# DoHoonKim8/halo2-lasso

Hardware: AMD Instinct MI355X
Metric: lasso_prove_time_ms (lower is better)
Workload: dtype u256 (BN254 Fr/Fq, 8x u32 Montgomery); 1 GPU; 2^24 AND Lasso lookup (32-bit operands, 4 chunks of 8+8 bits); lookups_per_proof=16777216, pcs=multilinear KZG (BN254), proof_bytes=64256, parallelism=1 GPU

## Files before the change

### bindings/rust/src/sys.rs

```rust
#![allow(non_camel_case_types, dead_code)]
use halo2_curves::bn256::{Fr, G1Affine, G2Affine};
use std::os::raw::{c_char, c_int, c_void};

pub type lh_status = c_int;
pub const LH_OK: lh_status = 0;
pub const LH_ERR_INVALID_SUMCHECK: lh_status = -1;
pub const LH_ERR_INVALID_PCS_PARAM: lh_status = -2;
pub const LH_ERR_INVALID_PCS_OPEN: lh_status = -3;
pub const LH_ERR_INVALID_SNARK: lh_status = -4;
pub const LH_ERR_SERIALIZATION: lh_status = -5;
pub const LH_ERR_TRANSCRIPT: lh_status = -6;
pub const LH_ERR_DEVICE: lh_status = -7;
pub const LH_ERR_ARG: lh_status = -8;

pub const LH_SC_MAX_TERMS: usize = 48;
pub const LH_SC_MAX_FACTORS: usize = 4;
pub const LH_SC_EVALUATIONS: c_int = 0;
pub const LH_SC_COEFFICIENTS: c_int = 1;
pub const LH_LASSO_MAX_CHUNKS: usize = 8;
pub const LH_LASSO_MAX_MEMORIES: usize = 16;
pub const LH_LASSO_MAX_TERMS: usize = 16;
pub const LH_RCCL_UNIQUE_ID_BYTES: usize = 128;

#[repr(C)] pub struct lh_ctx { _p: [u8; 0] }
// ... 71 lines not shown
    pub g_num_factors: [u8; LH_LASSO_MAX_TERMS],
    pub g_factor: [[u8; LH_SC_MAX_FACTORS]; LH_LASSO_MAX_TERMS],
}

#[repr(C)]
pub struct lh_comm {
    pub rank: c_int,
    pub size: c_int,
    pub user: *mut c_void,
    pub all_gather: Option<unsafe extern "C" fn(*mut c_void, *const c_void, *mut c_void, usize) -> c_int>,
    pub all_gather_device: Option<unsafe extern "C" fn(*mut c_void, *const c_void, *mut c_void, usize, *mut c_void) -> c_int>,
}

#[repr(C)]
pub struct lh_hp_lookup { pub inputs: *const lh_expr, pub tables: *const lh_expr, pub width: usize }
#[repr(C)] #[derive(Clone, Copy)]
pub struct lh_hp_lasso_lookup {
    pub table: lh_lasso_table,
    pub output_poly: usize,
    pub chunk_polys: [usize; LH_LASSO_MAX_CHUNKS],
}
#[repr(C)]
pub struct lh_hp_param {
    pub num_vars: usize,
    pub num_instance_polys: usize,
    pub num_instances: *const usize,
    pub num_preprocess_polys: usize,
    pub d_preprocess_polys: *const *const c_void,
    pub num_witness_polys: usize,
    pub num_challenges: usize,
    pub num_lookups: usize,
    pub lookups: *const lh_hp_lookup,
    pub num_permutation_polys: usize,
    pub permutation_poly_index: *const usize,
    pub d_permutation_polys: *const *const c_void,
    pub num_permutation_z_polys: usize,
    pub expression: lh_expr,
    pub num_lasso_lookups: usize,
    pub lasso_lookups: *const lh_hp_lasso_lookup,
}
#[repr(C)]
pub struct lh_hp_vparam {
    pub num_vars: usize,
    pub num_instance_polys: usize,
    pub num_instances: *const usize,
    pub num_witness_polys: usize,
    pub num_challenges: usize,
    pub num_lookups: usize,
    pub num_permutation_z_polys: usize,
    pub expression: lh_expr,
    pub num_preprocess_polys: usize,
    pub preprocess_comms: *const G1Affine,
    pub num_permutation_polys: usize,
    pub permutation_comms: *const G1Affine,
    pub num_lasso_lookups: usize,
    pub lasso_lookups: *const lh_hp_lasso_lookup,
}
#[repr(C)]
pub struct lh_hp_circuit {
    pub user: *mut c_void,
    pub synthesize: Option<unsafe extern "C" fn(*mut c_void, usize, *const Fr, usize, *mut *const c_void, usize) -> c_int>,
}

#[repr(C)]
#[derive(Clone, Copy, Debug, Default)]
pub struct lh_lasso_route {
    pub open_small_depth: u32,
    pub open_small_passes: u32,
    pub eq_factored_rounds: u32,
    pub standard_rounds: u32,
    pub rw_leaf_rounds: u32,
    pub resident_tails: u32,
    pub resident_rounds: u32,
    pub packed_ts_pairs: u32,
    pub derived_commitments: u32,
    pub sorted_dim_reuse: u32,
    pub sharded_rounds: u32,
    pub shard_exchanges: u32,
    pub window_table_jobs: u32,
    pub open_precommit: u32,
    pub resident_layers: u32,
    pub pp_folds: u32,
    pub msm_half_batches: u32,
    pub reserved: [u32; 7],
}

extern "C" {
    pub fn lh_last_error() -> *const c_char;
    pub fn lh_version() -> *const c_char;
    pub fn lh_ctx_create(device_id: c_int, out: *mut *mut lh_ctx) -> lh_status;
    pub fn lh_ctx_destroy(ctx: *mut lh_ctx);
    pub fn lh_ctx_sync(ctx: *mut lh_ctx) -> lh_status;
    pub fn lh_ctx_stream(ctx: *mut lh_ctx) -> *mut c_void;
    pub fn lh_alloc(ctx: *mut lh_ctx, bytes: usize, d_out: *mut *mut c_void) -> lh_status;
    pub fn lh_free(ctx: *mut lh_ctx, d_ptr: *mut c_void) -> lh_status;
    pub fn lh_upload(ctx: *mut lh_ctx, d_dst: *mut c_void, src: *const c_void, bytes: usize) -> lh_status;
    pub fn lh_download(ctx: *mut lh_ctx, dst: *mut c_void, d_src: *const c_void, bytes: usize) -> lh_status;
    pub fn lh_fr_from_u64(ctx: *mut lh_ctx, d_in: *const u64, n: usize, d_out: *mut Fr) -> lh_status;
    pub fn lh_fr_from_u32(ctx: *mut lh_ctx, d_in: *const u32, n: usize, d_out: *mut Fr) -> lh_status;
    pub fn lh_fr_batch_invert(ctx: *mut lh_ctx, d_in: *const Fr, n: usize, d_out: *mut Fr) -> lh_status;
    pub fn lh_fix_var(ctx: *mut lh_ctx, d_in: *const Fr, n_in: usize, x: *const Fr, d_out: *mut Fr) -> lh_status;
    pub fn lh_eq_xy(ctx: *mut lh_ctx, y: *const Fr, num_vars: usize, d_out: *mut Fr) -> lh_status;
    pub fn lh_evaluate(ctx: *mut lh_ctx, d_polys: *const *const Fr, num_polys: usize, num_vars: usize,
                       point: *const Fr, out_evals: *mut Fr) -> lh_status;
    pub fn lh_lincomb(ctx: *mut lh_ctx, d_polys: *const *const Fr, w: *const Fr, num_polys: usize, n: usize,
                      d_out: *mut Fr) -> lh_status;
    pub fn lh_sumcheck_prove(ctx: *mut lh_ctx, prover_kind: c_int, num_vars: usize, expr: *const lh_sop,
                             d_polys: *const *const Fr, num_polys: usize, ys: *const Fr, num_ys: usize,
                             sum: *const Fr, t: *mut lh_transcript, out_challenges: *mut Fr, out_evals: *mut Fr) -> lh_status;
    pub fn lh_sumcheck_prove_expr(ctx: *mut lh_ctx, num_vars: usize, expr: *const lh_expr, d_polys: *const *const Fr,
                                  num_polys: usize, challenges: *const Fr, num_challenges: usize, ys: *const Fr,
                                  num_ys: usize, sum: *const Fr, t: *mut lh_transcript, out_challenges: *mut Fr,
                                  out_evals: *mut Fr) -> lh_status;
    pub fn lh_sumcheck_verify(prover_kind: c_int, num_vars: usize, degree: usize, sum: *const Fr,
                              t: *mut lh_transcript, out_eval: *mut Fr, out_x: *mut Fr) -> lh_status;
    pub fn lh_gkr_fractional_prove(ctx: *mut lh_ctx, num_batching: usize, num_vars: usize,
                                   claimed_p_0s: *const *const Fr, claimed_q_0s: *const *const Fr,
                                   d_ps: *const *const Fr, d_qs: *const *const Fr, t: *mut lh_transcript,
                                   out_p_xs: *mut Fr, out_q_xs: *mut Fr, out_x: *mut Fr) -> lh_status;
    pub fn lh_msm(ctx: *mut lh_ctx, d_scalars: *const Fr, d_bases: *const G1Affine, n: usize, out: *mut G1Affine) -> lh_status;
    pub fn lh_msm_u32(ctx: *mut lh_ctx, d_scalars: *const u32, d_bases: *const G1Affine, n: usize, out: *mut G1Affine) -> lh_status;
    pub fn lh_srs_upload(ctx: *mut lh_ctx, eqs_flat: *const G1Affine, num_vars: usize, out: *mut *mut lh_srs) -> lh_status;
    pub fn lh_srs_num_vars(srs: *const lh_srs) -> usize;
    pub fn lh_srs_free(ctx: *mut lh_ctx, srs: *mut lh_srs);
    pub fn lh_mkzg_batch_commit(ctx: *mut lh_ctx, srs: *const lh_srs, d_polys: *const *const Fr, num_polys: usize,
                                num_vars: usize, out_comms: *mut G1Affine) -> lh_status;
    pub fn lh_mkzg_open(ctx: *mut lh_ctx, srs: *const lh_srs, d_poly: *const Fr, num_vars: usize, point: *const Fr,
                        t: *mut lh_transcript, out_eval: *mut Fr) -> lh_status;
    pub fn lh_mkzg_batch_open(ctx: *mut lh_ctx, srs: *const lh_srs, num_vars: usize, d_polys: *const *const Fr,
                              num_polys: usize, points: *const Fr, num_points: usize, evals: *const lh_evaluation,
                              num_evals: usize, t: *mut lh_transcript) -> lh_status;
    pub fn lh_mkzg_vp_new(g1: *const G1Affine, g2: *const G2Affine, ss: *const G2Affine, num_vars: usize,
                          out: *mut *mut lh_mkzg_vp) -> lh_status;
    pub fn lh_mkzg_vp_free(vp: *mut lh_mkzg_vp);
    pub fn lh_mkzg_verify(vp: *const lh_mkzg_vp, comm: *const G1Affine, point: *const Fr, num_vars: usize,
                          eval: *const Fr, t: *mut lh_transcript) -> lh_status;
    pub fn lh_mkzg_batch_verify(vp: *const lh_mkzg_vp, num_vars: usize, comms: *const G1Affine, num_comms: usize,
                                points: *const Fr, num_points: usize, evals: *const lh_evaluation, num_evals: usize,
                                t: *mut lh_transcript) -> lh_status;
    pub fn lh_lasso_prove(ctx: *mut lh_ctx, srs: *const lh_srs, table: *const lh_lasso_table, num_vars: usize,
                          d_dims: *const *const u32, t: *mut lh_transcript) -> lh_status;
    pub fn lh_lasso_verify(vp: *const lh_mkzg_vp, table: *const lh_lasso_table, num_vars: usize,
                           t: *mut lh_transcript) -> lh_status;
    pub fn lh_ctx_set_comm(ctx: *mut lh_ctx, comm: *const lh_comm, shard_bit: usize) -> lh_status;
    pub fn lh_rccl_unique_id(out: *mut u8) -> lh_status;
    pub fn lh_ctx_set_comm_rccl(ctx: *mut lh_ctx, rank: c_int, size: c_int, unique_id: *const u8, shard_bit: usize) -> lh_status;
    pub fn lh_ctx_set_comm_loopback(ctx: *mut lh_ctx, rank: c_int, size: c_int, shard_bit: usize) -> lh_status;
    pub fn lh_ctx_comm_stats(ctx: *mut lh_ctx, out: *mut u64) -> lh_status;
    pub fn lh_ctx_comm_phase_stats(ctx: *mut lh_ctx, out: *mut u64, reset: c_int) -> lh_status;
    pub fn lh_ctx_memory_stats(ctx: *mut lh_ctx, out: *mut u64) -> lh_status;
    pub fn lh_ctx_host_cpus(ctx: *mut lh_ctx, bus_id: *mut c_char, bus_id_cap: usize, cpulist: *mut c_char, cpulist_cap: usize) -> lh_status;
    pub fn lh_shard_extract(ctx: *mut lh_ctx, d_global: *const c_void, n_local: usize, shard_bit: usize, rho: usize,
                            rank: usize, elem_bytes: usize, d_local: *mut c_void) -> lh_status;
    pub fn lh_ctx_set_option(ctx: *mut lh_ctx, name: *const c_char, value: i64) -> lh_status;
    pub fn lh_ctx_get_option(ctx: *mut lh_ctx, name: *const c_char, out: *mut i64) -> lh_status;
    pub fn lh_lasso_last_route(ctx: *mut lh_ctx, out: *mut lh_lasso_route) -> lh_status;
    pub fn lh_lasso_prove_sharded(ctx: *mut lh_ctx, srs: *const lh_srs, table: *const lh_lasso_table, num_vars: usize,
                                  d_dims_local: *const *const u32, t: *mut lh_transcript) -> lh_status;
    pub fn lh_hyperplonk_prove(ctx: *mut lh_ctx, srs: *const lh_srs, pp: *const lh_hp_param,
                               instances: *const *const Fr, d_witness_polys: *const *const Fr,
                               t: *mut lh_transcript) -> lh_status;
    pub fn lh_hyperplonk_prove_sharded(ctx: *mut lh_ctx, srs: *const lh_srs, pp: *const lh_hp_param,
                                       instances: *const *const Fr, d_witness_polys_local: *const *const Fr,
                                       t: *mut lh_transcript) -> lh_status;
    pub fn lh_hyperplonk_prove_phases(ctx: *mut lh_ctx, srs: *const lh_srs, pp: *const lh_hp_param, num_phases: usize,
                                      num_witness_polys: *const usize, num_challenges: *const usize,
                                      instances: *const *const Fr, circuit: *const lh_hp_circuit,
// ... 135 lines not shown
```

### halo2-lasso_amd/__init__.py

```python
import ctypes as C

from . import _ffi
from ._ffi import (lh_fr, lh_g1, lh_sop, lh_evaluation, lh_lasso_table, lh_transcript,
                   LH_SC_EVALUATIONS, LH_SC_COEFFICIENTS)

R_MOD = 0x30644E72E131A029B85045B68181585D2833E84879B9709143E1F593F0000001
Q_MOD = 0x30644E72E131A029B85045B68181585D97816A916871CA8D3C208C16D87CFD47
_MONT = 1 << 256
_MONT_INV_R = pow(_MONT, -1, R_MOD)
_MONT_INV_Q = pow(_MONT, -1, Q_MOD)

SUBTABLE_IDENTITY, SUBTABLE_AND, SUBTABLE_XOR = 0, 1, 2


class Error(Exception):
    code = None


class InvalidSumcheck(Error):
    code = _ffi.LH_ERR_INVALID_SUMCHECK


class InvalidPcsParam(Error):
    code = _ffi.LH_ERR_INVALID_PCS_PARAM
# ... 335 lines not shown
    return _fr_list(out, len(polys))


EvaluationsProver = LH_SC_EVALUATIONS
CoefficientsProver = LH_SC_COEFFICIENTS


class SumOfProducts:

    def __init__(self, terms, global_eq=-1):
        self.terms, self.global_eq = [(c % R_MOD, list(f)) for c, f in terms], global_eq

    def to_c(self):
        s = lh_sop()
        s.num_terms, s.global_eq = len(self.terms), self.global_eq
        for m, (coeff, facs) in enumerate(self.terms):
            C.memmove(C.byref(s.coeff[m]), fr_to_bytes(coeff), 32)
            s.num_factors[m] = len(facs)
            for k, f in enumerate(facs):
                s.factor[m][k] = f
        return s


class ClassicSumCheck:
    @staticmethod
    def prove(ctx, prover, num_vars, expression, polys, ys, sum_, transcript):
        if len(expression.terms) > _ffi.LH_SC_MAX_TERMS:
            raise ArgumentError("too many terms")
        ys_flat = [v for y in ys for v in y]
        ch = (lh_fr * max(num_vars, 1))()
        ev = (lh_fr * max(len(polys), 1))()
        sop = expression.to_c()
        _check(ctx.lib.lh_sumcheck_prove(ctx.h, prover, num_vars, C.byref(sop), _ptr_array(polys), len(polys),
                                         _fr_array(ys_flat), len(ys), _fr_array([sum_]), transcript.p, ch, ev))
        return _fr_list(ch, num_vars), _fr_list(ev, len(polys))


def sum_check_prove_expression(ctx, num_vars, expression, polys, challenges, ys, sum_, transcript):
    ce, keep = expression.to_c()
    ys_flat = [v for y in ys for v in y]
    ch = (lh_fr * max(num_vars, 1))()
    ev = (lh_fr * max(len(polys), 1))()
    _check(ctx.lib.lh_sumcheck_prove_expr(ctx.h, num_vars, C.byref(ce), _ptr_array(polys), len(polys),
                                          _fr_array(challenges), len(challenges), _fr_array(ys_flat), len(ys),
                                          _fr_array([sum_]), transcript.p, ch, ev))
    return _fr_list(ch, num_vars), _fr_list(ev, len(polys))


def prove_fractional_sum_check(ctx, claimed_p_0s, claimed_q_0s, ps, qs, transcript):
    B = len(ps)
    if not (B == len(qs) == len(claimed_p_0s) == len(claimed_q_0s)):
        raise ArgumentError("length mismatch")
    num_vars = ps[0].num_vars if B else 0
    for p in list(ps) + list(qs):
        if p.num_vars != num_vars:
            raise ArgumentError("num_vars mismatch")

    def opt(claims):
        keep = [_fr_array([c]) if c is not None else None for c in claims]
        arr = (C.POINTER(lh_fr) * max(B, 1))()
        for i, k in enumerate(keep):
            arr[i] = C.cast(k, C.POINTER(lh_fr)) if k is not None else None
        return arr, keep

    cp, keep_p = opt(claimed_p_0s)
    cq, keep_q = opt(claimed_q_0s)
    p_xs, q_xs, x = (lh_fr * max(B, 1))(), (lh_fr * max(B, 1))(), (lh_fr * max(num_vars, 1))()
    _check(ctx.lib.lh_gkr_fractional_prove(ctx.h, B, num_vars, cp, cq, _ptr_array(ps), _ptr_array(qs),
                                           transcript.p, p_xs, q_xs, x))
    return _fr_list(p_xs, B), _fr_list(q_xs, B), _fr_list(x, num_vars)


def prove_grand_product(ctx, leaves, transcript):
    B = len(leaves)
    nv = (C.c_size_t * max(B, 1))(*[p.num_vars for p in leaves])
    total = sum(p.num_vars for p in leaves)
    roots, claims, points = (lh_fr * max(B, 1))(), (lh_fr * max(B, 1))(), (lh_fr * max(total, 1))()
    _check(ctx.lib.lh_grand_product_prove(ctx.h, B, _ptr_array(leaves), nv, transcript.p, roots, claims, points))
    pts, flat, off = [], _fr_list(points, total), 0
    for p in leaves:
        pts.append(flat[off:off + p.num_vars])
        off += p.num_vars
    return _fr_list(roots, B), list(zip(_fr_list(claims, B), pts))


def variable_base_msm(ctx, scalars, bases, n=None):
    n = len(scalars) if n is None else n
    out = lh_g1()
    _check(ctx.lib.lh_msm(ctx.h, scalars.ptr, bases.ptr, n, C.byref(out)))
    return g1_from_bytes(bytes(out))


def variable_base_msm_u32(ctx, scalars, bases, n):
    out = lh_g1()
    _check(ctx.lib.lh_msm_u32(ctx.h, scalars.ptr, bases.ptr, n, C.byref(out)))
    return g1_from_bytes(bytes(out))


class Evaluation:

    def __init__(self, poly, point, value):
        self.poly, self.point, self.value = poly, point, value % R_MOD


class MultilinearKzgParams:
    def __init__(self, ctx, handle, borrowed=False):
        self.ctx, self.h, self.borrowed = ctx, handle, borrowed

    def view(self, ctx):
        return MultilinearKzgParams(ctx, self.h, borrowed=True)

    @property
    def num_vars(self):
        return self.ctx.lib.lh_srs_num_vars(self.h)

    def eqs_bytes(self):
        total = (2 << self.num_vars) - 1
        out = C.create_string_buffer(64 * total)
        _check(self.ctx.lib.lh_srs_download(self.ctx.h, self.h, out))
        return out.raw

    def eqs(self):
        n = self.num_vars
        total = (2 << n) - 1
        out = C.create_string_buffer(64 * total)
        _check(self.ctx.lib.lh_srs_download(self.ctx.h, self.h, out))
        pts = [g1_from_bytes(out.raw[64 * i:64 * i + 64]) for i in range(total)]
        return [pts[(1 << k) - 1:(2 << k) - 1] for k in range(n + 1)]

    def free(self):
        if self.h and self.ctx.h and not self.borrowed:
            self.ctx.lib.lh_srs_free(self.ctx.h, self.h)
        self.h = None

    def __del__(self):
        try:
            self.free()
        except Exception:
            pass


class MultilinearKzg:

    @staticmethod
    def setup(ctx, ss):
        h = C.c_void_p()
        _check(ctx.lib.lh_mkzg_setup(ctx.h, _fr_array(ss), len(ss), C.byref(h)))
        return MultilinearKzgParams(ctx, h)

    @staticmethod
    def upload(ctx, eqs_levels):
        flat = b"".join(g1_to_bytes(p) for lvl in eqs_levels for p in lvl)
        return MultilinearKzg.upload_bytes(ctx, flat, len(eqs_levels) - 1)

    @staticmethod
    def upload_bytes(ctx, eqs_flat, num_vars):
        if len(eqs_flat) != 64 * ((2 << num_vars) - 1):
            raise ArgumentError("flat SRS has the wrong length")
        h = C.c_void_p()
        _check(ctx.lib.lh_srs_upload(ctx.h, eqs_flat, num_vars, C.byref(h)))
        return MultilinearKzgParams(ctx, h)

    @staticmethod
    def commit(pp, poly):
        out = lh_g1()
        _check(pp.ctx.lib.lh_mkzg_commit(pp.ctx.h, pp.h, poly.ptr, poly.num_vars, C.byref(out)))
# ... 859 lines not shown
                return _ffi.LH_ERR_ARG
            C.memmove(recv, out, len(out))
            return 0
        except Exception:
            return _ffi.LH_ERR_DEVICE
    comm = _ffi.lh_comm()
    comm.rank, comm.size, comm.user = rank, size, None
    comm.all_gather = _ffi._AG_CB(cb)
    ctx._comm_keepalive = (comm, cb)
    _check(ctx.lib.lh_ctx_set_comm(ctx.h, C.byref(comm), shard_bit))


def rccl_unique_id():
    buf = C.create_string_buffer(_ffi.LH_RCCL_UNIQUE_ID_BYTES)
    _check(_ffi.load().lh_rccl_unique_id(buf))
    return buf.raw


def attach_comm_rccl(ctx, rank, size, unique_id, shard_bit):
    if len(unique_id) != _ffi.LH_RCCL_UNIQUE_ID_BYTES:
        raise ArgumentError("unique id must be %d bytes" % _ffi.LH_RCCL_UNIQUE_ID_BYTES)
    _check(ctx.lib.lh_ctx_set_comm_rccl(ctx.h, rank, size, unique_id, shard_bit))


def comm_stats(ctx):
    out = (C.c_uint64 * 2)()
    _check(ctx.lib.lh_ctx_comm_stats(ctx.h, out))
    return {"device": int(out[0]), "host": int(out[1])}


def comm_phase_stats(ctx, reset=False):
    out = (C.c_uint64 * 16)()
    _check(ctx.lib.lh_ctx_comm_phase_stats(ctx.h, out, 1 if reset else 0))
    names = ["witness", "commit", "surge", "leaves", "gkr", "evals", "open", "outside"]
    return {nm: {"collectives": int(out[2 * i]), "bytes": int(out[2 * i + 1])} for i, nm in enumerate(names) if out[2 * i]}


def memory_stats(ctx):
    out = (C.c_uint64 * 4)()
    _check(ctx.lib.lh_ctx_memory_stats(ctx.h, out))
    return {"arena_high_water_bytes": int(out[0]), "arena_reserved_bytes": int(out[1]), "device_free_bytes": int(out[2]),
            "device_total_bytes": int(out[3])}


def attach_comm_loopback(ctx, rank, size, shard_bit):
    _check(ctx.lib.lh_ctx_set_comm_loopback(ctx.h, rank, size, shard_bit))


def detach_comm(ctx):
    _check(ctx.lib.lh_ctx_set_comm(ctx.h, None, 0))
    ctx._comm_keepalive = None


def shard_of(column, rank, size, shard_bit):
    rho = size.bit_length() - 1
    n = len(column)
    return column.reshape(n >> (shard_bit + rho), size, 1 << shard_bit)[:, rank, :].reshape(-1).copy()


def shard_poly(poly, rank, size, shard_bit):
    rho = size.bit_length() - 1
    n_local = (1 << poly.num_vars) >> rho
    out = poly.ctx.alloc(32 * n_local)
    _check(poly.ctx.lib.lh_shard_extract(poly.ctx.h, poly.ptr, n_local, shard_bit, rho, rank, 32, out.ptr))
    return MultilinearPolynomial(poly.ctx, out, poly.num_vars - rho)


def lasso_prove_sharded(pp, table, num_vars, dims_local, transcript):
    if len(dims_local) != table.c:
        raise ArgumentError("expected %d dim columns" % table.c)
    t = table.to_c()
    _check(pp.ctx.lib.lh_lasso_prove_sharded(pp.ctx.h, pp.h, C.byref(t), num_vars, _ptr_array(dims_local), transcript.p))


def lasso_last_timing(ctx):
    out = (C.c_double * _ffi.LH_LASSO_NUM_PHASES)()
    _check(ctx.lib.lh_lasso_last_timing(ctx.h, out))
    names = ["witness", "commit", "surge", "leaves", "gkr", "evals", "open_n", "open_l", "total"]
    return dict(zip(names, list(out)))


ROUTE_FIELDS = ["open_small_depth", "open_small_passes", "eq_factored_rounds", "standard_rounds", "rw_leaf_rounds",
                "resident_tails", "resident_rounds", "packed_ts_pairs", "derived_commitments", "sorted_dim_reuse",
                "sharded_rounds", "shard_exchanges", "window_table_jobs", "open_precommit", "resident_layers", "pp_folds", "msm_half_batches"]


def lasso_last_route(ctx):
    out = (C.c_uint32 * 24)()
    _check(ctx.lib.lh_lasso_last_route(ctx.h, out))
    return dict(zip(ROUTE_FIELDS, [int(v) for v in out]))


def set_option(ctx, name, value):
    _check(ctx.lib.lh_ctx_set_option(ctx.h, name.encode(), int(value)))


def get_option(ctx, name):
    out = C.c_int64(0)
    _check(ctx.lib.lh_ctx_get_option(ctx.h, name.encode(), C.byref(out)))
    return int(out.value)


def profile_enable(ctx, on=True):
    _check(ctx.lib.lh_profile_enable(ctx.h, int(on)))


def profile_read(ctx):
    n = C.c_size_t()
    _check(ctx.lib.lh_profile_read(ctx.h, None, 0, C.byref(n)))
    arr = (_ffi.lh_prof_rec * max(n.value, 1))()
    _check(ctx.lib.lh_profile_read(ctx.h, arr, n.value, C.byref(n)))
    return [dict(name=r.name.decode(), ms=r.ms, bytes=r.bytes, muls=r.muls, items=r.items) for r in arr[:n.value]]


from . import expression
```

### halo2-lasso_amd/_ffi.py

```python
import ctypes as C
import os

_HERE = os.path.dirname(os.path.abspath(__file__))
LIB_PATH = os.path.join(_HERE, "liblasso_hip.so")

LH_OK = 0
LH_ERR_INVALID_SUMCHECK, LH_ERR_INVALID_PCS_PARAM, LH_ERR_INVALID_PCS_OPEN = -1, -2, -3
LH_ERR_INVALID_SNARK, LH_ERR_SERIALIZATION, LH_ERR_TRANSCRIPT, LH_ERR_DEVICE, LH_ERR_ARG = -4, -5, -6, -7, -8
LH_SC_EVALUATIONS, LH_SC_COEFFICIENTS = 0, 1
LH_SC_MAX_TERMS, LH_SC_MAX_FACTORS = 48, 4
LH_LASSO_MAX_CHUNKS, LH_LASSO_MAX_MEMORIES, LH_LASSO_MAX_TERMS = 8, 16, 16
LH_LASSO_NUM_PHASES = 9


class lh_fr(C.Structure):
    _fields_ = [("l", C.c_uint64 * 4)]


class lh_g1(C.Structure):
    _fields_ = [("x", C.c_uint64 * 4), ("y", C.c_uint64 * 4)]


class lh_sop(C.Structure):
    _fields_ = [("num_terms", C.c_uint32), ("global_eq", C.c_int32),
# ... 62 lines not shown
class lh_evaluation(C.Structure):
    _fields_ = [("poly", C.c_uint32), ("point", C.c_uint32), ("value", lh_fr)]


_AG_CB = C.CFUNCTYPE(C.c_int, C.c_void_p, C.c_void_p, C.c_void_p, C.c_size_t)
_AGD_CB = C.CFUNCTYPE(C.c_int, C.c_void_p, C.c_void_p, C.c_void_p, C.c_size_t, C.c_void_p)
LH_RCCL_UNIQUE_ID_BYTES = 128


class lh_comm(C.Structure):
    _fields_ = [("rank", C.c_int), ("size", C.c_int), ("user", C.c_void_p), ("all_gather", _AG_CB),
                ("all_gather_device", _AGD_CB)]


class lh_prof_rec(C.Structure):
    _fields_ = [("name", C.c_char * 40), ("ms", C.c_double), ("bytes", C.c_double), ("muls", C.c_double),
                ("items", C.c_double)]


_FE_CB = C.CFUNCTYPE(C.c_int, C.c_void_p, C.POINTER(lh_fr))
_G1_CB = C.CFUNCTYPE(C.c_int, C.c_void_p, C.POINTER(lh_g1))


class lh_transcript(C.Structure):
    _fields_ = [("user", C.c_void_p),
                ("write_field_element", _FE_CB), ("common_field_element", _FE_CB),
                ("squeeze_challenge", _FE_CB),
                ("write_commitment", _G1_CB), ("common_commitment", _G1_CB),
                ("read_field_element", _FE_CB), ("read_commitment", _G1_CB)]


_HASH_W_CB = C.CFUNCTYPE(C.c_int, C.c_void_p, C.POINTER(C.c_uint8))


class lh_hash_transcript(C.Structure):
    _fields_ = [("user", C.c_void_p), ("write_hash", _HASH_W_CB), ("read_hash", _HASH_W_CB)]


class lh_g2(C.Structure):
    _fields_ = [("x_c0", C.c_uint64 * 4), ("x_c1", C.c_uint64 * 4), ("y_c0", C.c_uint64 * 4), ("y_c1", C.c_uint64 * 4)]


_P = C.c_void_p
_SZ = C.c_size_t
SIGNATURES = {
    "lh_last_error": (C.c_char_p, []),
    "lh_version": (C.c_char_p, []),
    "lh_ctx_create": (C.c_int, [C.c_int, C.POINTER(_P)]),
    "lh_ctx_destroy": (None, [_P]),
    "lh_ctx_sync": (C.c_int, [_P]),
    "lh_ctx_stream": (_P, [_P]),
    "lh_alloc": (C.c_int, [_P, _SZ, C.POINTER(_P)]),
    "lh_free": (C.c_int, [_P, _P]),
    "lh_upload": (C.c_int, [_P, _P, _P, _SZ]),
    "lh_download": (C.c_int, [_P, _P, _P, _SZ]),
    "lh_keccak_transcript_new": (C.c_int, [C.POINTER(C.POINTER(lh_transcript))]),
    "lh_keccak_transcript_free": (None, [C.POINTER(lh_transcript)]),
    "lh_keccak_transcript_proof": (C.c_int, [C.POINTER(lh_transcript), C.POINTER(C.POINTER(C.c_uint8)),
                                             C.POINTER(_SZ)]),
    "lh_fr_from_u64": (C.c_int, [_P, _P, _SZ, _P]),
    "lh_fr_from_u32": (C.c_int, [_P, _P, _SZ, _P]),
    "lh_fr_to_repr": (C.c_int, [_P, _P, _SZ, _P]),
    "lh_fr_from_repr": (C.c_int, [_P, _P, _SZ, _P]),
    "lh_fr_add": (C.c_int, [_P, _P, _P, _SZ, _P]),
    "lh_fr_sub": (C.c_int, [_P, _P, _P, _SZ, _P]),
    "lh_fr_mul": (C.c_int, [_P, _P, _P, _SZ, _P]),
    "lh_fr_mul_chain": (C.c_int, [_P, _P, _P, _SZ, C.c_int, _P]),
    "lh_fr_batch_invert": (C.c_int, [_P, _P, _SZ, _P]),
    "lh_fix_var": (C.c_int, [_P, _P, _SZ, C.POINTER(lh_fr), _P]),
    "lh_eq_xy": (C.c_int, [_P, C.POINTER(lh_fr), _SZ, _P]),
    "lh_evaluate": (C.c_int, [_P, C.POINTER(_P), _SZ, _SZ, C.POINTER(lh_fr), C.POINTER(lh_fr)]),
    "lh_lincomb": (C.c_int, [_P, C.POINTER(_P), C.POINTER(lh_fr), _SZ, _SZ, _P]),
    "lh_sumcheck_prove": (C.c_int, [_P, C.c_int, _SZ, C.POINTER(lh_sop), C.POINTER(_P), _SZ,
                                    C.POINTER(lh_fr), _SZ, C.POINTER(lh_fr), C.POINTER(lh_transcript),
                                    C.POINTER(lh_fr), C.POINTER(lh_fr)]),
    "lh_sumcheck_prove_expr": (C.c_int, [_P, _SZ, C.POINTER(lh_expr), C.POINTER(_P), _SZ, C.POINTER(lh_fr), _SZ,
                                         C.POINTER(lh_fr), _SZ, C.POINTER(lh_fr), C.POINTER(lh_transcript),
                                         C.POINTER(lh_fr), C.POINTER(lh_fr)]),
    "lh_gkr_fractional_prove": (C.c_int, [_P, _SZ, _SZ, C.POINTER(C.POINTER(lh_fr)), C.POINTER(C.POINTER(lh_fr)),
                                          C.POINTER(_P), C.POINTER(_P), C.POINTER(lh_transcript),
                                          C.POINTER(lh_fr), C.POINTER(lh_fr), C.POINTER(lh_fr)]),
    "lh_grand_product_prove": (C.c_int, [_P, _SZ, C.POINTER(_P), C.POINTER(_SZ), C.POINTER(lh_transcript),
                                         C.POINTER(lh_fr), C.POINTER(lh_fr), C.POINTER(lh_fr)]),
    "lh_msm": (C.c_int, [_P, _P, _P, _SZ, C.POINTER(lh_g1)]),
    "lh_msm_u32": (C.c_int, [_P, _P, _P, _SZ, C.POINTER(lh_g1)]),
    "lh_mkzg_setup": (C.c_int, [_P, C.POINTER(lh_fr), _SZ, C.POINTER(_P)]),
    "lh_srs_upload": (C.c_int, [_P, _P, _SZ, C.POINTER(_P)]),
    "lh_srs_download": (C.c_int, [_P, _P, _P]),
    "lh_srs_num_vars": (_SZ, [_P]),
    "lh_srs_free": (None, [_P, _P]),
    "lh_mkzg_commit": (C.c_int, [_P, _P, _P, _SZ, C.POINTER(lh_g1)]),
    "lh_mkzg_batch_commit": (C.c_int, [_P, _P, C.POINTER(_P), _SZ, _SZ, C.POINTER(lh_g1)]),
    "lh_mkzg_open": (C.c_int, [_P, _P, _P, _SZ, C.POINTER(lh_fr), C.POINTER(lh_transcript), C.POINTER(lh_fr)]),
    "lh_mkzg_batch_open": (C.c_int, [_P, _P, _SZ, C.POINTER(_P), _SZ, C.POINTER(lh_fr), _SZ,
                                     C.POINTER(lh_evaluation), _SZ, C.POINTER(lh_transcript)]),
    "lh_lasso_prove": (C.c_int, [_P, _P, C.POINTER(lh_lasso_table), _SZ, C.POINTER(_P), C.POINTER(lh_transcript)]),
    "lh_lasso_last_timing": (C.c_int, [_P, C.POINTER(C.c_double)]),
    "lh_ctx_set_option": (C.c_int, [_P, C.c_char_p, C.c_int64]),
    "lh_ctx_get_option": (C.c_int, [_P, C.c_char_p, C.POINTER(C.c_int64)]),
    "lh_lasso_last_route": (C.c_int, [_P, C.POINTER(C.c_uint32)]),
    "lh_ctx_set_comm": (C.c_int, [_P, C.POINTER(lh_comm), _SZ]),
    "lh_rccl_unique_id": (C.c_int, [C.c_char_p]),
    "lh_ctx_set_comm_rccl": (C.c_int, [_P, C.c_int, C.c_int, C.c_char_p, _SZ]),
    "lh_ctx_set_comm_loopback": (C.c_int, [_P, C.c_int, C.c_int, _SZ]),
    "lh_ctx_comm_stats": (C.c_int, [_P, C.POINTER(C.c_uint64)]),
    "lh_ctx_comm_phase_stats": (C.c_int, [_P, C.POINTER(C.c_uint64), C.c_int]),
    "lh_ctx_memory_stats": (C.c_int, [_P, C.POINTER(C.c_uint64)]),
    "lh_ctx_host_cpus": (C.c_int, [_P, C.c_char_p, C.c_size_t, C.c_char_p, C.c_size_t]),
    "lh_lasso_prove_sharded": (C.c_int, [_P, _P, C.POINTER(lh_lasso_table), _SZ, C.POINTER(_P),
                                         C.POINTER(lh_transcript)]),
    "lh_hyperplonk_prove": (C.c_int, [_P, _P, C.POINTER(lh_hp_param), C.POINTER(C.POINTER(lh_fr)), C.POINTER(_P),
                                      C.POINTER(lh_transcript)]),
    "lh_shard_extract": (C.c_int, [_P, _P, _SZ, _SZ, _SZ, _SZ, _SZ, _P]),
    "lh_hyperplonk_prove_sharded": (C.c_int, [_P, _P, C.POINTER(lh_hp_param), C.POINTER(C.POINTER(lh_fr)), C.POINTER(_P),
                                              C.POINTER(lh_transcript)]),
    "lh_hyperplonk_prove_phases": (C.c_int, [_P, _P, C.POINTER(lh_hp_param), _SZ, C.POINTER(_SZ), C.POINTER(_SZ),
                                             C.POINTER(C.POINTER(lh_fr)), C.POINTER(lh_hp_circuit),
                                             C.POINTER(lh_transcript)]),
    "lh_hyperplonk_verify_phases": (C.c_int, [_P, C.POINTER(lh_hp_vparam), _SZ, C.POINTER(_SZ), C.POINTER(_SZ),
                                              C.POINTER(C.POINTER(lh_fr)), C.POINTER(lh_transcript)]),
    "lh_keccak_transcript_from_proof": (C.c_int, [C.c_char_p, _SZ, C.POINTER(C.POINTER(lh_transcript))]),
    "lh_keccak_transcript_remaining": (C.c_int, [C.POINTER(lh_transcript), C.POINTER(_SZ)]),
    "lh_mkzg_vp_setup": (C.c_int, [C.POINTER(lh_fr), _SZ, C.POINTER(_P)]),
    "lh_mkzg_vp_new": (C.c_int, [C.POINTER(lh_g1), C.POINTER(lh_g2), C.POINTER(lh_g2), _SZ, C.POINTER(_P)]),
    "lh_mkzg_vp_export": (C.c_int, [_P, C.POINTER(lh_g1), C.POINTER(lh_g2), C.POINTER(lh_g2)]),
    "lh_mkzg_vp_num_vars": (_SZ, [_P]),
    "lh_mkzg_vp_free": (None, [_P]),
    "lh_pairing_check": (C.c_int, [C.POINTER(lh_g1), C.POINTER(lh_g2), _SZ, C.POINTER(C.c_int)]),
    "lh_mkzg_verify": (C.c_int, [_P, C.POINTER(lh_g1), C.POINTER(lh_fr), _SZ, C.POINTER(lh_fr),
                                 C.POINTER(lh_transcript)]),
    "lh_mkzg_batch_verify": (C.c_int, [_P, _SZ, C.POINTER(lh_g1), _SZ, C.POINTER(lh_fr), _SZ,
                                       C.POINTER(lh_evaluation), _SZ, C.POINTER(lh_transcript)]),
    "lh_sumcheck_verify": (C.c_int, [C.c_int, _SZ, _SZ, C.POINTER(lh_fr), C.POINTER(lh_transcript),
                                     C.POINTER(lh_fr), C.POINTER(lh_fr)]),
    "lh_lasso_verify": (C.c_int, [_P, C.POINTER(lh_lasso_table), _SZ, C.POINTER(lh_transcript)]),
    "lh_hyperplonk_verify": (C.c_int, [_P, C.POINTER(lh_hp_vparam), C.POINTER(C.POINTER(lh_fr)),
                                       C.POINTER(lh_transcript)]),
    "lh_ukzg_setup": (C.c_int, [_P, C.POINTER(lh_fr), _SZ, C.POINTER(_P)]),
    "lh_usrs_upload": (C.c_int, [_P, C.c_char_p, _SZ, C.POINTER(_P)]),
    "lh_usrs_download": (C.c_int, [_P, _P, C.c_char_p]),
    "lh_usrs_size": (_SZ, [_P]),
    "lh_usrs_free": (None, [_P, _P]),
    "lh_zeromorph_batch_commit": (C.c_int, [_P, _P, _SZ, C.POINTER(_P), _SZ, _SZ, C.POINTER(lh_g1)]),
    "lh_zeromorph_open": (C.c_int, [_P, _P, _SZ, _P, _SZ, C.POINTER(lh_fr), C.POINTER(lh_transcript)]),
    "lh_zeromorph_batch_open": (C.c_int, [_P, _P, _SZ, _SZ, C.POINTER(_P), _SZ, C.POINTER(lh_fr), _SZ,
                                          C.POINTER(lh_evaluation), _SZ, C.POINTER(lh_transcript)]),
    "lh_zeromorph_vp_setup": (C.c_int, [C.POINTER(lh_fr), _SZ, _SZ, C.POINTER(_P)]),
    "lh_zeromorph_vp_new": (C.c_int, [C.POINTER(lh_g1), C.POINTER(lh_g2), C.POINTER(lh_g2), C.POINTER(lh_g2),
                                      C.POINTER(_P)]),
    "lh_zeromorph_vp_export": (C.c_int, [_P, C.POINTER(lh_g1), C.POINTER(lh_g2), C.POINTER(lh_g2), C.POINTER(lh_g2)]),
    "lh_zeromorph_vp_free": (None, [_P]),
    "lh_zeromorph_verify": (C.c_int, [_P, C.POINTER(lh_g1), C.POINTER(lh_fr), _SZ, C.POINTER(lh_fr),
                                      C.POINTER(lh_transcript)]),
    "lh_zeromorph_batch_verify": (C.c_int, [_P, _SZ, C.POINTER(lh_g1), _SZ, C.POINTER(lh_fr), _SZ,
                                            C.POINTER(lh_evaluation), _SZ, C.POINTER(lh_transcript)]),
    "lh_lasso_prove_zeromorph": (C.c_int, [_P, _P, _SZ, C.POINTER(lh_lasso_table), _SZ, C.POINTER(_P),
                                           C.POINTER(lh_transcript)]),
    "lh_lasso_verify_zeromorph": (C.c_int, [_P, C.POINTER(lh_lasso_table), _SZ, C.POINTER(lh_transcript)]),
    "lh_hyperplonk_prove_zeromorph": (C.c_int, [_P, _P, _SZ, C.POINTER(lh_hp_param), C.POINTER(C.POINTER(lh_fr)),
                                                C.POINTER(_P), C.POINTER(lh_transcript)]),
    "lh_hyperplonk_verify_zeromorph": (C.c_int, [_P, C.POINTER(lh_hp_vparam), C.POINTER(C.POINTER(lh_fr)),
                                                 C.POINTER(lh_transcript)]),
    "lh_hyperplonk_prove_phases_zeromorph": (C.c_int, [_P, _P, _SZ, C.POINTER(lh_hp_param), _SZ, C.POINTER(_SZ),
                                                       C.POINTER(_SZ), C.POINTER(C.POINTER(lh_fr)),
                                                       C.POINTER(lh_hp_circuit), C.POINTER(lh_transcript)]),
    "lh_hyperplonk_verify_phases_zeromorph": (C.c_int, [_P, C.POINTER(lh_hp_vparam), _SZ, C.POINTER(_SZ), C.POINTER(_SZ),
# ... 117 lines not shown
```

### halo2-lasso_amd/csrc/capi.cpp

```cpp
#include "host.hpp"
#include "brakedown.hpp"
#include <memory>

using namespace lh;

struct lh_ctx {
  Ctx c;
};
struct lh_srs {
  Srs s;
};
struct lh_mkzg_vp {
  VerifierParams* p;
};
struct lh_usrs {
  USrs s;
};
struct lh_zm_vp {
  ZmVerifierParams* p;
};
struct lh_ukzg_vp {
  UkzgVerifierParams* p;
};
struct lh_ipa_param {
// ... 319 lines not shown
  NEED_N(w, num_polys);
  NEED_N(d_out, n);
  k_lincomb(ctx->c, (const Fr* const*)d_polys, (const Fr*)w, num_polys, n, (Fr*)d_out);
  LH_CATCH
}

lh_status lh_sumcheck_prove(lh_ctx* ctx, int prover_kind, size_t num_vars, const lh_sop* expr,
                            const lh_fr* const* d_polys, size_t num_polys, const lh_fr* ys, size_t num_ys,
                            const lh_fr* sum, lh_transcript* t, lh_fr* out_challenges, lh_fr* out_evals) {
  LH_TRY NEED_CTX(ctx);
  NEED(expr);
  NEED(sum);
  NEED_N(d_polys, num_polys);
  NEED_N(ys, num_ys);
  LH_REQUIRE(prover_kind == LH_SC_EVALUATIONS || prover_kind == LH_SC_COEFFICIENTS, LH_ERR_ARG, "bad prover kind");
  Transcript tr(t);
  HFr s;
  memcpy(&s, sum, 32);
  SumCheckResult r = sum_check_prove(ctx->c, prover_kind, num_vars, *expr, (const Fr* const*)d_polys, num_polys,
                                     (const HFr*)ys, num_ys, s, tr);
  if (out_challenges) memcpy(out_challenges, r.challenges.data(), r.challenges.size() * 32);
  if (out_evals) memcpy(out_evals, r.evals.data(), r.evals.size() * 32);
  LH_CATCH
}

lh_status lh_sumcheck_prove_expr(lh_ctx* ctx, size_t num_vars, const lh_expr* expr, const lh_fr* const* d_polys,
                                 size_t num_polys, const lh_fr* challenges, size_t num_challenges, const lh_fr* ys,
                                 size_t num_ys, const lh_fr* sum, lh_transcript* t, lh_fr* out_challenges,
                                 lh_fr* out_evals) {
  LH_TRY NEED_CTX(ctx);
  NEED(expr);
  NEED(sum);
  NEED_N(d_polys, num_polys);
  NEED_N(challenges, num_challenges);
  NEED_N(ys, num_ys);
  Transcript tr(t);
  HFr s;
  memcpy(&s, sum, 32);
  SumCheckResult r = sum_check_prove_expr(ctx->c, num_vars, *expr, (const Fr* const*)d_polys, num_polys,
                                          (const HFr*)challenges, num_challenges, (const HFr*)ys, num_ys, s, tr);
  if (out_challenges) memcpy(out_challenges, r.challenges.data(), r.challenges.size() * 32);
  if (out_evals) memcpy(out_evals, r.evals.data(), r.evals.size() * 32);
  LH_CATCH
}

lh_status lh_gkr_fractional_prove(lh_ctx* ctx, size_t num_batching, size_t num_vars,
                                  const lh_fr* const* claimed_p_0s, const lh_fr* const* claimed_q_0s,
                                  const lh_fr* const* d_ps, const lh_fr* const* d_qs, lh_transcript* t,
                                  lh_fr* out_p_xs, lh_fr* out_q_xs, lh_fr* out_x) {
  LH_TRY NEED_CTX(ctx);
  NEED_N(claimed_p_0s, num_batching);
  NEED_N(claimed_q_0s, num_batching);
  NEED_N(d_ps, num_batching);
  NEED_N(d_qs, num_batching);
  Transcript tr(t);
  FracSumCheckResult r =
      prove_fractional_sum_check(ctx->c, num_batching, num_vars, (const HFr* const*)claimed_p_0s,
                                 (const HFr* const*)claimed_q_0s, (const Fr* const*)d_ps, (const Fr* const*)d_qs, tr);
  if (out_p_xs) memcpy(out_p_xs, r.p_xs.data(), r.p_xs.size() * 32);
  if (out_q_xs) memcpy(out_q_xs, r.q_xs.data(), r.q_xs.size() * 32);
  if (out_x) memcpy(out_x, r.x.data(), r.x.size() * 32);
  LH_CATCH
}

lh_status lh_grand_product_prove(lh_ctx* ctx, size_t num_trees, const lh_fr* const* d_leaves, const size_t* num_vars,
                                 lh_transcript* t, lh_fr* out_roots, lh_fr* out_claims, lh_fr* out_points) {
  LH_TRY NEED_CTX(ctx);
  NEED(num_vars);
  NEED_N(d_leaves, num_trees);
  Transcript tr(t);
  GrandProductResult r = prove_grand_product(ctx->c, num_trees, (const Fr* const*)d_leaves, num_vars, tr);
  if (out_roots) memcpy(out_roots, r.roots.data(), num_trees * 32);
  if (out_claims) memcpy(out_claims, r.claims.data(), num_trees * 32);
  if (out_points) {
    lh_fr* p = out_points;
    for (size_t b = 0; b < num_trees; b++) {
      memcpy(p, r.points[b].data(), r.points[b].size() * 32);
      p += r.points[b].size();
    }
  }
  LH_CATCH
}

lh_status lh_msm(lh_ctx* ctx, const lh_fr* d_scalars, const lh_g1* d_bases, size_t n, lh_g1* out) {
  LH_TRY NEED_CTX(ctx);
  NEED(out);
  NEED_N(d_scalars, n);
  NEED_N(d_bases, n);
  MsmJob job{d_scalars, false, (const G1Affine*)d_bases, n};
  msm_batch(ctx->c, &job, 1, (G1Affine*)out);
  LH_CATCH
}
lh_status lh_msm_u32(lh_ctx* ctx, const uint32_t* d_scalars, const lh_g1* d_bases, size_t n, lh_g1* out) {
  LH_TRY NEED_CTX(ctx);
  NEED(out);
  NEED_N(d_scalars, n);
  NEED_N(d_bases, n);
  MsmJob job{d_scalars, true, (const G1Affine*)d_bases, n};
  msm_batch(ctx->c, &job, 1, (G1Affine*)out);
  LH_CATCH
}

lh_status lh_mkzg_setup(lh_ctx* ctx, const lh_fr* ss, size_t num_vars, lh_srs** out) {
  LH_TRY NEED_CTX(ctx);
  NEED(out);
  NEED_N(ss, num_vars);
  Srs* s = mkzg_setup(ctx->c, (const HFr*)ss, num_vars);
  lh_srs* w = new lh_srs();
  w->s = *s;
  delete s;
  *out = w;
  LH_CATCH
}
lh_status lh_srs_upload(lh_ctx* ctx, const lh_g1* eqs_flat, size_t num_vars, lh_srs** out) {
  LH_TRY NEED_CTX(ctx);
  NEED(out);
  NEED(eqs_flat);
  LH_REQUIRE(num_vars < 31, LH_ERR_ARG, "srs: num_vars too large");
  std::unique_ptr<lh_srs> w(new lh_srs());
  w->s.num_vars = num_vars;
  size_t total = ((size_t)2 << num_vars) - 1;
  LH_HIP(hipMalloc((void**)&w->s.d_eqs, total * sizeof(G1Affine)));
  if (hipMemcpyAsync(w->s.d_eqs, eqs_flat, total * sizeof(G1Affine), hipMemcpyHostToDevice, ctx->c.stream) != hipSuccess ||
      hipStreamSynchronize(ctx->c.stream) != hipSuccess) {
    (void)hipFree(w->s.d_eqs);
    throw lh::Error(LH_ERR_DEVICE, "srs upload failed");
  }
  *out = w.release();
  LH_CATCH
}
lh_status lh_srs_download(lh_ctx* ctx, const lh_srs* srs, lh_g1* eqs_flat) {
  LH_TRY NEED_CTX(ctx);
  NEED(srs);
  NEED(eqs_flat);
  size_t total = ((size_t)2 << srs->s.num_vars) - 1;
  LH_HIP(hipMemcpyAsync(eqs_flat, srs->s.d_eqs, total * sizeof(G1Affine), hipMemcpyDeviceToHost, ctx->c.stream));
  ctx->c.sync();
  LH_CATCH
}
size_t lh_srs_num_vars(const lh_srs* srs) { return srs ? srs->s.num_vars : 0; }
void lh_srs_free(lh_ctx* ctx, lh_srs* srs) {
  if (!srs) return;
  if (ctx) (void)hipStreamSynchronize(ctx->c.stream);
  if (srs->s.d_eqs) {
    (void)hipFree(srs->s.d_eqs);
  }
  for (G1Affine* p : srs->s.shard_levels)
    if (p) {
      (void)hipFree(p);
    }
  for (auto& kv : srs->s.win_tables)
    if (kv.second.d) (void)hipFree(kv.second.d);
  delete srs;
}

lh_status lh_mkzg_commit(lh_ctx* ctx, const lh_srs* srs, const lh_fr* d_poly, size_t num_vars, lh_g1* out) {
  LH_TRY NEED_CTX(ctx);
  NEED(srs);
  NEED(d_poly);
  NEED(out);
  const Fr* p = (const Fr*)d_poly;
  std::vector<HG1> c = mkzg_batch_commit(ctx->c, srs->s, &p, 1, num_vars);
  memcpy(out, c.data(), 64);
  LH_CATCH
}
lh_status lh_mkzg_batch_commit(lh_ctx* ctx, const lh_srs* srs, const lh_fr* const* d_polys, size_t num_polys,
// ... 1325 lines not shown
```

### halo2-lasso_amd/csrc/dev.hpp

```cpp
#pragma once
#include <hip/hip_runtime_api.h>
#include <stdint.h>
#include <stdarg.h>
#include <stdio.h>
#include <functional>
#include <string>
#include <vector>
#include <utility>
#include <stdexcept>

#include "../../include/lasso_hip.h"
#include "ec.cuh"

namespace lh {

struct Error : std::exception {
  int code;
  std::string msg;
  Error(int c, std::string m) : code(c), msg(std::move(m)) {}
  const char* what() const noexcept override { return msg.c_str(); }
};

void set_last_error(const char* msg);

// ... 22 lines not shown
    return (T*)alloc(n * sizeof(T));
  }
  Mark mark() const { return {cur_, blocks_.empty() ? 0 : blocks_[cur_].used}; }
  void release(Mark m);
  size_t high_water() const { return high_; }
  size_t reserved() const {
    size_t t = 0;
    for (const Block& b : blocks_) t += b.size;
    return t;
  }

 private:
  struct Block {
    char* p;
    size_t size, used;
  };
  std::vector<Block> blocks_;
  size_t cur_ = 0, high_ = 0;
};

struct ArenaScope {
  Arena& a;
  Arena::Mark m;
  explicit ArenaScope(Arena& a_) : a(a_), m(a_.mark()) {}
  ~ArenaScope() { a.release(m); }
};

struct ProfRec {
  char name[40];
  double ms;
  double bytes;
  double muls;
  double items;
};

struct ScFinishArgs {
  uint32_t* ticket;
  uint32_t last_ticket;
  Fr* out_host;
  uint32_t* flag;
  uint32_t seq;
  uint64_t* wide;
  uint32_t tag;
  uint64_t* lanes;
};
constexpr uint32_t FIN_LANE_SUMS = 65536;
constexpr unsigned SC_LANE_TAG_SHIFT = 40;

struct Options {
  int64_t open_small_min_vars = 21;
  bool open_small_min_vars_forced = false;
  int64_t open_small_depth = 0;
  int64_t sc_eq_factoring = 1;
  int64_t lasso_pack_ts = 1;
  int64_t sc_tail = 1;
  int64_t sc_tail_max_len = 8192;
  int64_t shard_exchange_log = 19;
  int64_t open_precommit = 1;
  int64_t msm_window_tables = 0;
  int64_t sc_pp_fold = 1;
  int64_t msm_half_batches = 1;
  int64_t gkr_resident = 1;
  int64_t comm_round = 0;
  Options();
  int64_t* find(const char* name);
  static bool in_range(const char* name, int64_t value);
};

enum class Knob {
  SC_TAIL_G, MSM_C_OFF, MSM_C_MAX, MSM_K2, MSM_SEG, MSM_SLAB_LOG, MSM_TREE_MAX, MSM_QUAD_MAX, MSM_TWO_LEVEL, MSM_HALF_MIN_LOG,
  MSM_HALF_COVER, EXPR_MONOMIALS, EXPR_JIT_MIN_VARS, EXPR_EF_MIN_VARS,
  FIN_LANES_MIN_BYTES, SC_U32, OPEN_U32_ROUNDS, OPEN_FOLD_COLS,
  HOST_THREADS, JIT_CACHE, JIT_CACHE_DIR, EXPR_JIT, SC_TAIL_TIMEOUT_MS, GKR_START_TIMEOUT_MS, COMM_WAIT_TIMEOUT_MS, COMM_A2A,
  COMM_PROBE,
  HOST_TRACE, SC_TAIL_TRACE, GKR_TRACE, SC_DEBUG, MSM_DEBUG, HP_DEBUG, COMM_DEBUG, OPEN_SMALL_CHECK,
  COMM_A2A_SELF, COMM_PROBE_FAIL, SHARDED_COUNTERS_MIN_R,
  COUNT
};
double knob(Knob k);
const char* knob_text(Knob k);
struct RouteStats {
  uint32_t v[LH_LASSO_ROUTE_WORDS] = {0};
  enum { OPEN_DEPTH, OPEN_PASSES, EF_ROUNDS, STD_ROUNDS, RW_ROUNDS, TAILS, TAIL_ROUNDS, PACKED_TS, DERIVED, SORTED_REUSE,
         SHARDED_ROUNDS, SHARD_EXCHANGES, WIN_TABLE_JOBS, OPEN_PRECOMMIT, RESIDENT_LAYERS, PP_FOLDS, MSM_HALF_BATCHES };
};

class HostWorker {
 public:
  HostWorker();
  ~HostWorker();
  void submit(std::function<void()> fn);
  void wait();
 private:
  struct Impl;
  Impl* impl_;
};

struct OpenPrecommit;
struct Ctx {
  Options opt;
  RouteStats route;
  int device = 0;
  hipStream_t stream = nullptr;
  Arena arena;
  void* pinned = nullptr;
  size_t pinned_bytes = 0;
  int num_cus = 256;
  int wall_clock_khz = 100000;
  double lasso_ms[LH_LASSO_NUM_PHASES] = {0};
  lh_comm comm = {0, 1, nullptr, nullptr, nullptr};
  bool has_comm = false;
  bool comm_loopback = false;
  size_t shard_bit = 0;
  bool shard_active = false;
  void* rccl_comm = nullptr;
  void* comm_stage = nullptr;
  size_t comm_stage_bytes = 0;
  uint64_t comm_stats[2] = {0, 0};
  uint64_t comm_phase_stats[8][2] = {};
  int comm_phase = 7;
  Fr* sc_redirect = nullptr;
  uint64_t* sc_wide = nullptr;
  uint32_t sc_tag = 0;
  uint32_t sc_tag_seq = 0;
  uint64_t* lanes_host = nullptr;
  bool comm_host_recv_ok = true;
  Fr* round_out(Fr* out_host) const { return sc_redirect ? sc_redirect : out_host; }
  void wait_round(uint32_t seq) {
    if (!sc_redirect) wait_flag(seq);
  }
  uint64_t* tail_trace = nullptr;
  std::vector<std::pair<const char*, double>> host_stamps;
  bool host_trace_on = false;
  void host_stamp(const char* tag);
  void host_stamps_print();
  struct EqHalfEntry {
    std::vector<uint8_t> key;
    const Fr* table;
    bool sharded = false;
  };
  std::vector<EqHalfEntry> eq_half_cache;
  bool prof = false;
  std::vector<ProfRec> prof_recs;
  bool live = false;
  struct LiveRec {
    ProfRec rec;
    hipEvent_t e0, e1;
    uint32_t batch;
  };
  std::vector<LiveRec> live_recs;
  std::vector<hipEvent_t> live_pool;
  uint32_t live_batch = 0;
  hipEvent_t live_event();
  void live_resolve(std::vector<ProfRec>& out);
  bool is_helper = false;
  Ctx* helper = nullptr;
  lh_ctx* helper_handle = nullptr;
  OpenPrecommit* precommit = nullptr;
  HostWorker* worker = nullptr;
  hipEvent_t handoff_ev = nullptr;
  hipEvent_t phase_ev[LH_LASSO_NUM_PHASES] = {};
  bool phase_ev_pending = false;
  void phase_times_resolve();
  hipEvent_t prof_ev[2] = {nullptr, nullptr};
  void* pin(size_t bytes);
  void* stage = nullptr;
  size_t stage_bytes = 0;
// ... 51 lines not shown
    while (((size_t)1 << rho) < R) rho++;
  }
  bool sharded(size_t num_vars) const { return on && num_vars >= j + (rho ? rho : 1) + 1; }
  size_t local_vars(size_t num_vars) const { return sharded(num_vars) ? num_vars - rho : num_vars; }
  size_t local_len(size_t num_vars) const { return (size_t)1 << local_vars(num_vars); }
};

struct ReplicatedRange {
  size_t first = 0, count = 0;
  ReplicatedRange(const Shard& sh, size_t len) {
    if (!sh.on || sh.R <= 1) {
      count = len;
    } else if (len < sh.R) {
      count = sh.rank == 0 || sh.loopback ? len : 0;
    } else {
      const size_t per = len / sh.R;
      first = sh.rank * per;
      count = sh.rank + 1 == sh.R ? len - first : per;
    }
  }
};

void host_parallel_for(size_t n, const std::function<void(size_t)>& fn);
void host_parallel_prewake(size_t n, unsigned us);

struct ProfScope {
  Ctx& c;
  ProfRec rec;
  bool on;
  ProfScope(Ctx& c_, const char* name, double bytes, double muls, double items) : c(c_), on(c_.prof) {
    if (!on) return;
    snprintf(rec.name, sizeof rec.name, "%s", name);
    rec.bytes = bytes, rec.muls = muls, rec.items = items, rec.ms = 0;
    if (!c.prof_ev[0]) {
      LH_HIP(hipEventCreate(&c.prof_ev[0]));
      LH_HIP(hipEventCreate(&c.prof_ev[1]));
    }
    LH_HIP(hipEventRecord(c.prof_ev[0], c.stream));
  }
  ~ProfScope() {
    if (!on) return;
    (void)hipEventRecord(c.prof_ev[1], c.stream);
    (void)hipEventSynchronize(c.prof_ev[1]);
    float ms = 0;
    (void)hipEventElapsedTime(&ms, c.prof_ev[0], c.prof_ev[1]);
    rec.ms = ms;
    c.prof_recs.push_back(rec);
  }
};

void k_fr_from_u64(Ctx&, const uint64_t* in, size_t n, Fr* out);
void k_fr_from_u32(Ctx&, const uint32_t* in, size_t n, Fr* out);
void k_fr_to_repr(Ctx&, const Fr* in, size_t n, Fr* out);
void k_fr_from_repr(Ctx&, const Fr* in, size_t n, Fr* out);
void k_fr_binop(Ctx&, int op, const Fr* a, const Fr* b, size_t n, Fr* out);
void k_fr_mul_chain(Ctx&, const Fr* a, const Fr* b, size_t n, int iters, Fr* out);
void k_fr_batch_invert(Ctx&, const Fr* in, size_t n, Fr* out);
void k_fix_var(Ctx&, const Fr* in, size_t n_in, const Fr& x, Fr* out);
void k_fix_var_multi(Ctx&, const Fr* const* in, Fr* const* out, size_t count, size_t n_in, const Fr& x);
void k_eq_xy(Ctx&, const Fr* y, size_t num_vars, Fr* out);
void k_bind_first(Ctx&, const Fr* const* in, size_t count, const Fr& x, Fr* out_host);
void k_gather_heads(Ctx&, const Fr* const* in, size_t count, int k, Fr* out_host);
void k_lincomb(Ctx&, const Fr* const* polys, const Fr* w, size_t count, size_t n, Fr* out);
void k_lincomb_fold(Ctx&, const Fr* const* polys, const Fr* w, size_t count, size_t half, const Fr& x, Fr* out);
bool k_lincomb_fold_small(Ctx&, const uint32_t* const* cols, const size_t* lens, const Fr* coef, size_t count, size_t half,
                          const Fr& x, Fr* out);
void k_inner_products(Ctx&, const Fr* const* polys, size_t count, const Fr* weights, size_t n, Fr* out_host);
void k_inner_products_u32(Ctx&, const uint32_t* const* polys, size_t count, const Fr* weights, size_t n,
                          Fr* out_host);
void k_inner_products_small(Ctx&, const uint32_t* const* polys, size_t count, const Fr* weights, size_t n, Fr* out_host);
void k_inner_products_small_half(Ctx&, const uint32_t* const* polys, size_t count, const Fr* eq_half, size_t half,
                                 const Fr& y0, Fr* out_host);
void k_inner_products_small_quads(Ctx&, const uint32_t* col, const Fr* e0, size_t quads, Fr* out_host);
void k_inner_products_quads(Ctx&, const uint32_t* const* cols, const size_t* lens, size_t count, const Fr* e1, size_t quads,
                            Fr* d_out);
void k_lincomb_bind2(Ctx&, const uint32_t* const* cols, const size_t* lens, const Fr* w, size_t count, const Fr& r0, const Fr& r1,
                     const Fr* eq_level, size_t size, Fr* out, Fr* out_host);
void k_sc_round_u32_bind2(Ctx&, const uint32_t* col, const Fr* eq_level, const Fr& r0, const Fr& r1, size_t size, Fr* out,
                          Fr* out_host);
void k_lincomb_mixed(Ctx&, const Fr* const* fr, const Fr* wfr, size_t num_fr, const uint32_t* const* sm,
                     const size_t* sm_len, const Fr* wsm, size_t num_sm, size_t n, Fr* out);
void k_tree_up(Ctx&, const Fr* in, size_t half, Fr* out);
void k_tree_up_multi(Ctx&, const Fr* const* in, Fr* const* out, size_t count, size_t half);
void k_tree_tops(Ctx&, const Fr* const* in, Fr* const* out, const int* H, size_t count);
void k_frac_up(Ctx&, const Fr* p, const Fr* q, size_t half, Fr* vp, Fr* vq);
void k_quotient_step(Ctx&, const Fr* rem, size_t half, const Fr& x, Fr* q, Fr* rem_out);
void k_lasso_rw_leaves(Ctx&, const uint32_t* dim, const uint32_t* e, const uint32_t* ts, size_t n,
                       const Fr& gamma, const Fr& gamma2, const Fr& tau, Fr* rs, Fr* ws);
void k_lasso_rw_leaves_up(Ctx&, const uint32_t* dim, const uint32_t* e, const uint32_t* ts, size_t n, const Fr& gamma,
                          const Fr& gamma2, const Fr& tau, Fr* rs, Fr* ws, Fr* rs_up, Fr* ws_up);
void k_lasso_if_leaves(Ctx&, int subtable, uint32_t chunk_bits, const uint32_t* final_cts, size_t m,
                       const Fr& gamma, const Fr& gamma2, const Fr& tau, Fr* init, Fr* fin);
void k_or_u32(Ctx&, const uint32_t* const* cols, size_t count, size_t n, uint32_t* out_host);
void k_fill_u32(Ctx&, uint32_t* out, uint32_t value, size_t n);
void k_pack_u32(Ctx&, const uint32_t* a, const uint32_t* b, uint32_t shift, size_t n, uint32_t* out);
void k_delta_u32(Ctx&, const uint32_t* col, size_t len, size_t half, uint64_t offset, uint32_t* out_lo, uint32_t* out_hi);
void k_lasso_counters(Ctx&, const uint32_t* const* dims, size_t cc, size_t n, size_t m, uint32_t* const* read_ts,
                      uint32_t* const* final_cts, uint32_t* const* keep_sorted = nullptr, uint32_t* const* keep_index = nullptr);
void k_cs_partition(Ctx&, const uint32_t* const* dims, size_t cc, size_t n, size_t m, unsigned rho, unsigned j, unsigned hi_bits,
                    uint32_t* const* sidx, uint32_t* const* send, uint32_t* start_host, bool* bad_out);
void k_cs_rank(Ctx&, const uint32_t* const* recv, const size_t* n_recv, size_t cc, unsigned hi_bits, unsigned a_bits, size_t m_loc,
               uint32_t* const* ret, uint32_t* counts);
void k_cs_scatter(Ctx&, const uint32_t* const* back, const uint32_t* const* sidx, size_t cc, size_t n, uint32_t* const* read_ts);
void k_cs_final(Ctx&, const uint32_t* all_counts, size_t cc, size_t m, unsigned rho, size_t m_loc, uint32_t* const* final_cts);
void k_lasso_subtable_read(Ctx&, int subtable, uint32_t chunk_bits, const uint32_t* dim, size_t n, uint32_t* e);
struct LassoG {
  uint32_t num_terms;
  Fr coeff[LH_LASSO_MAX_TERMS];
  uint8_t nfac[LH_LASSO_MAX_TERMS];
  uint8_t fac[LH_LASSO_MAX_TERMS][LH_SC_MAX_FACTORS];
  const uint32_t* e[LH_LASSO_MAX_MEMORIES];
};
void k_lasso_output(Ctx&, const LassoG& g, size_t n, Fr* a);
struct LassoGSmall {
  uint32_t num_terms;
  uint32_t coeff[LH_LASSO_MAX_TERMS];
  uint8_t fac[LH_LASSO_MAX_TERMS];
  const uint32_t* e[LH_LASSO_MAX_MEMORIES];
};
void k_lasso_output_small(Ctx&, const LassoGSmall& g, size_t n, uint32_t* a);
bool k_fr_to_index(Ctx&, const Fr* in, size_t n, uint32_t bits, uint32_t* out);
bool k_fr_tables_equal(Ctx&, const Fr* a, const Fr* b, size_t n);

void rccl_unique_id(uint8_t out[LH_RCCL_UNIQUE_ID_BYTES]);
void comm_attach_rccl(Ctx&, int rank, int size, const uint8_t id[LH_RCCL_UNIQUE_ID_BYTES], size_t shard_bit);
void comm_probe_host_recv(Ctx&);
void comm_attach_loopback(Ctx&, int rank, int size, size_t shard_bit);
void comm_detach(Ctx&);
void comm_all_gather_dev(Ctx&, const void* d_send, void* d_recv, size_t bytes);
void comm_all_gather_host(Ctx&, const void* send, void* recv, size_t bytes);
void comm_all_to_all_multi(Ctx&, size_t nbuf, const void* const* d_send, const size_t* send_off, const size_t* send_cnt,
                           void* const* d_recv, const size_t* recv_off, const size_t* recv_cnt, const size_t* peer_off,
                           const void* send_base, size_t send_stride, size_t elem);
void comm_sum_publish(Ctx&, const Fr* d_part, Fr* d_scratch, size_t count, Fr* out_host, uint32_t seq);
void comm_sum_lanes(Ctx&, uint64_t* d_lanes, uint64_t* d_scratch, size_t count, Fr* out_host);
uint32_t comm_next_tag(Ctx&);
void k_loopback_allreduce_lanes(Ctx&, const uint64_t* d_in, size_t n, size_t R, uint64_t* out);

void k_shard_merge(Ctx&, const void* gathered, size_t n_local, size_t j, size_t rho, size_t elem, void* global);
void k_gather_interleave(Ctx&, const Fr* gathered, size_t count, size_t n_local, size_t R, size_t block, Fr* const* out);
void k_sum_publish(Ctx&, const Fr* all, size_t R, size_t D, Fr* out_host, uint32_t seq);
void k_shard_extract(Ctx&, const void* global, size_t n_local, size_t j, size_t rho, size_t s, size_t elem, void* local);
void k_loopback_gather(Ctx&, const void* d_send, void* d_recv, size_t bytes, size_t R);
void k_scale(Ctx&, const Fr* in, const Fr& w, size_t n, Fr* out);

constexpr int SC_MAX_TABLES = 72;
struct ScRound {
  const Fr* in[SC_MAX_TABLES];
  Fr* out[SC_MAX_TABLES];
  uint32_t num_tables;
  uint32_t num_terms;
  int32_t global_eq;
  Fr coeff[LH_SC_MAX_TERMS];
  uint8_t coeff_is_one[LH_SC_MAX_TERMS];
  uint8_t nfac[LH_SC_MAX_TERMS];
  uint8_t fac[LH_SC_MAX_TERMS][LH_SC_MAX_FACTORS];
  Fr r;
  const Fr* eq_level;
  uint8_t pp;
};
bool k_sc_round(Ctx&, const ScRound& rd, int degree, bool bind, size_t size, Fr* evals_host);
bool k_sc_round_streams(const ScRound& rd, int degree, size_t size);
void k_eq_levels(Ctx&, const Fr* in, size_t n_in, Fr* const* levels, size_t nlev);
constexpr int SC_OPEN_MAX_TERMS = 6;
struct ScOpenRound {
  const Fr* in[SC_OPEN_MAX_TERMS];
  Fr* out[SC_OPEN_MAX_TERMS];
  const Fr* eq_level[SC_OPEN_MAX_TERMS];
  uint32_t num_terms;
  Fr r;
};
void k_sc_round_open(Ctx&, const ScOpenRound& rd, bool bind, size_t size, Fr* out_host);

// ... 200 lines not shown
```

### halo2-lasso_amd/csrc/gkr.cpp

```cpp
#include <algorithm>
#include <functional>
#include <chrono>
#include <memory>
#include <thread>
#include "host.hpp"
#include "resident_host.hpp"

namespace lh {

FracSumCheckResult prove_fractional_sum_check(Ctx& c, size_t B, size_t num_vars, const HFr* const* claimed_p_0s,
                                              const HFr* const* claimed_q_0s, const Fr* const* d_ps,
                                              const Fr* const* d_qs, Transcript& tr) {
  LH_REQUIRE(B != 0, LH_ERR_ARG, "fractional sum-check: num_batching == 0");
  LH_REQUIRE(num_vars >= 1, LH_ERR_ARG, "fractional sum-check: num_vars == 0");
  LH_REQUIRE(3 * B <= LH_SC_MAX_TERMS && 4 * B + 1 <= (size_t)SC_MAX_TABLES, LH_ERR_ARG,
             "fractional sum-check: too many fractions for one round kernel");
  ArenaScope scope(c.arena);
  std::vector<std::vector<const Fr*>> lp(num_vars), lq(num_vars);
  for (size_t b = 0; b < B; b++) {
    lp[0].push_back(d_ps[b]);
    lq[0].push_back(d_qs[b]);
  }
  for (size_t h = 1; h < num_vars; h++) {
    size_t half = (size_t)1 << (num_vars - h);
// ... 6 lines not shown
    }
  }
  std::vector<HFr> top(4 * B);
  {
    std::vector<const Fr*> heads;
    for (size_t b = 0; b < B; b++) {
      heads.push_back(lp[num_vars - 1][b]);
      heads.push_back(lq[num_vars - 1][b]);
    }
    Fr* out = (Fr*)c.pin(2 * SC_MAX_TABLES * sizeof(Fr));
    k_gather_heads(c, heads.data(), heads.size(), 2, out);
    memcpy(top.data(), out, 4 * B * sizeof(Fr));
  }
  std::vector<HFr> claimed_p(B), claimed_q(B);
  for (size_t b = 0; b < B; b++) {
    const HFr &p_l = top[4 * b], &p_r = top[4 * b + 1], &q_l = top[4 * b + 2], &q_r = top[4 * b + 3];
    claimed_p[b] = p_l * q_r + p_r * q_l;
    claimed_q[b] = q_l * q_r;
  }
  for (size_t b = 0; b < B; b++) {
    if (claimed_p_0s && claimed_p_0s[b]) tr.common_field_element(claimed_p[b]);
    else tr.write_field_element(claimed_p[b]);
  }
  for (size_t b = 0; b < B; b++) {
    if (claimed_q_0s && claimed_q_0s[b]) tr.common_field_element(claimed_q[b]);
    else tr.write_field_element(claimed_q[b]);
  }

  std::vector<HFr> y;
  for (size_t h = num_vars; h-- > 0;) {
    const size_t nv = num_vars - 1 - h;
    const size_t half = (size_t)1 << nv;
    std::vector<HFr> x, evals;
    if (nv == 0) {
      evals = top;
    } else {
      HFr gamma = tr.squeeze_challenge();
      HFr claim = HFr::zero(), power = HFr::one();
      lh_sop expr;
      memset(&expr, 0, sizeof(expr));
      expr.global_eq = 0;
      std::vector<const Fr*> polys;
      for (size_t b = 0; b < B; b++) {
        claim += claimed_p[b] * power;
        HFr g_even = power;
        power *= gamma;
        claim += claimed_q[b] * power;
        HFr g_odd = power;
        power *= gamma;
        uint8_t p_l = 4 * b, p_r = 4 * b + 1, q_l = 4 * b + 2, q_r = 4 * b + 3;
        uint32_t m = expr.num_terms;
        memcpy(&expr.coeff[m], &g_even, 32);
        expr.num_factors[m] = 2, expr.factor[m][0] = p_l, expr.factor[m][1] = q_r;
        memcpy(&expr.coeff[m + 1], &g_even, 32);
        expr.num_factors[m + 1] = 2, expr.factor[m + 1][0] = p_r, expr.factor[m + 1][1] = q_l;
        memcpy(&expr.coeff[m + 2], &g_odd, 32);
        expr.num_factors[m + 2] = 2, expr.factor[m + 2][0] = q_l, expr.factor[m + 2][1] = q_r;
        expr.num_terms += 3;
        polys.push_back(lp[h][b]);
        polys.push_back(lp[h][b] + half);
        polys.push_back(lq[h][b]);
        polys.push_back(lq[h][b] + half);
      }
      ScOptions so;
      so.sum_is_exact = true;
      SumCheckResult sc = sum_check_prove(c, LH_SC_EVALUATIONS, nv, expr, polys.data(), polys.size(), y.data(), 1,
                                          claim, tr, so);
      x = sc.challenges;
      evals = sc.evals;
    }
    tr.write_field_elements(evals);
    HFr mu = tr.squeeze_challenge();
    for (size_t b = 0; b < B; b++) {
      const HFr &p_l = evals[4 * b], &p_r = evals[4 * b + 1], &q_l = evals[4 * b + 2], &q_r = evals[4 * b + 3];
      claimed_p[b] = p_l + mu * (p_r - p_l);
      claimed_q[b] = q_l + mu * (q_r - q_l);
    }
    x.push_back(mu);
    y = x;
  }
  return FracSumCheckResult{claimed_p, claimed_q, y};
}

GrandProductResult prove_grand_product(Ctx& c, size_t B, const Fr* const* d_leaves, const size_t* num_vars,
                                       Transcript& tr, const Fr* const* d_level_up, const uint8_t* plus_one,
                                       const std::function<void()>& trees_built) {
  LH_REQUIRE(B != 0, LH_ERR_ARG, "grand product: no trees");
  size_t max_depth = 0;
  for (size_t b = 0; b < B; b++) {
    LH_REQUIRE(num_vars[b] >= 1 && num_vars[b] < 32, LH_ERR_ARG, "grand product: every tree needs >= 2 leaves");
    max_depth = std::max(max_depth, num_vars[b]);
  }
  LH_REQUIRE(2 * B + 1 <= (size_t)SC_MAX_TABLES && B <= LH_SC_MAX_TERMS, LH_ERR_ARG,
             "grand product: too many trees for one round kernel");
  ArenaScope scope(c.arena);
  const Shard sh(c);
  std::vector<std::vector<const Fr*>> level(B);
  {
    const size_t SMALL = 9;
    std::vector<const Fr*> top_in(B);
    std::vector<Fr*> top_out(B);
    std::vector<int> top_H(B);
    std::vector<size_t> cur_h(B);
    size_t max_h = 0;
    for (size_t b = 0; b < B; b++) {
      level[b].resize(num_vars[b]);
      level[b][num_vars[b] - 1] = d_leaves[b];
      size_t h = num_vars[b] - 1;
      if (d_level_up && d_level_up[b] && h > SMALL && (!sh.on || sh.sharded(h))) {
        level[b][h - 1] = d_level_up[b];
        h--;
      }
      cur_h[b] = h;
      max_h = std::max(max_h, h);
    }
    for (size_t h = max_h; h >= 1 && (h > SMALL || sh.sharded(h + 1)); h--) {
      std::vector<const Fr*> ins;
      std::vector<Fr*> outs;
      std::vector<size_t> who;
      const bool in_sh = sh.sharded(h + 1), out_sh = sh.sharded(h);
      const size_t half = (size_t)1 << (in_sh ? h - sh.rho : h);
      for (size_t b = 0; b < B; b++) {
        if (cur_h[b] != h) continue;
        ins.push_back(level[b][h]);
        who.push_back(b);
        cur_h[b] = h - 1;
      }
      if (ins.empty()) continue;
      if (in_sh && !out_sh) {
        Fr* block = c.arena.alloc_n<Fr>(ins.size() * half);
        std::vector<Fr*> rep(ins.size());
        for (size_t k = 0; k < ins.size(); k++) {
          outs.push_back(block + k * half);
          rep[k] = c.arena.alloc_n<Fr>((size_t)1 << h);
        }
        k_tree_up_multi(c, ins.data(), outs.data(), ins.size(), half);
        comm_gather_tables(c, block, ins.size(), half, half, rep.data());
        c.route.v[RouteStats::SHARD_EXCHANGES]++;
        for (size_t k = 0; k < ins.size(); k++) level[who[k]][h - 1] = rep[k];
      } else {
        for (size_t k = 0; k < ins.size(); k++) {
          outs.push_back(c.arena.alloc_n<Fr>(half));
          level[who[k]][h - 1] = outs.back();
        }
        k_tree_up_multi(c, ins.data(), outs.data(), ins.size(), half);
      }
    }
    for (size_t b = 0; b < B; b++) {
      const size_t h = cur_h[b];
      LH_REQUIRE(h <= SMALL && !sh.sharded(h + 1), LH_ERR_ARG, "grand product: internal level mismatch");
      Fr* tops = c.arena.alloc_n<Fr>(((size_t)2 << h));
      top_in[b] = level[b][h];
      top_out[b] = tops;
      top_H[b] = (int)h;
      for (size_t k = 0; k < h; k++) level[b][k] = tops + (((size_t)2 << k) - 2);
    }
    k_tree_tops(c, top_in.data(), top_out.data(), top_H.data(), B);
  }
  std::vector<HFr> top(2 * B);
  {
    std::vector<const Fr*> heads;
    for (size_t b = 0; b < B; b++) heads.push_back(level[b][0]);
    Fr* out = (Fr*)c.pin(2 * SC_MAX_TABLES * sizeof(Fr));
    k_gather_heads(c, heads.data(), heads.size(), 2, out);
    memcpy(top.data(), out, 2 * B * sizeof(Fr));
  }
  GrandProductResult res;
  res.roots.resize(B);
  res.claims.resize(B);
  res.points.resize(B);
  for (size_t b = 0; b < B; b++) res.roots[b] = top[2 * b] * top[2 * b + 1];
  tr.write_field_elements(res.roots);

  std::vector<HFr> claims = res.roots, y;
  HFr resident_lam;
  bool have_resident_lam = false;
  GkrResident resident(c);
  std::vector<GkrLayerDev> resident_layers;
  if (c.opt.gkr_resident && c.opt.sc_tail && c.opt.sc_eq_factoring) {
    std::vector<GkrLayerDev> layers;
    for (size_t h = 1; h < max_depth; h++) {
      GkrLayerDev L;
      memset(&L, 0, sizeof(L));
      uint32_t nb = 0;
      bool ok = !sh.sharded(h + 1) && k_gkr_resident_geometry((uint32_t)h, &L.g, &L.s_log);
      bool any_leaf = false, all_leaf = true;
      for (size_t b = 0; b < B && ok; b++) {
        if (num_vars[b] <= h) continue;
        ok = nb < (uint32_t)GKR_MAX_TREES && level[b][h] != nullptr;
        if (!ok) break;
        any_leaf = any_leaf || num_vars[b] == h + 1;
        all_leaf = all_leaf && num_vars[b] == h + 1;
        L.lv[nb++] = level[b][h];
      }
      if (ok && plus_one && any_leaf && all_leaf) ok = false;
      if (!ok || nb == 0) break;
      L.h = (uint32_t)h, L.B = nb;
      layers.push_back(L);
    }
    resident_layers.swap(layers);
  }
  if (trees_built) trees_built();
  if (!resident_layers.empty()) resident.launch(resident_layers);
  for (size_t h = 0; h < max_depth; h++) {
    std::vector<size_t> active;
    for (size_t b = 0; b < B; b++)
      if (num_vars[b] > h) active.push_back(b);
    if (h >= 1 && resident.live && h <= resident.H) {
      HFr lam = tr.squeeze_challenge();
      HFr claim = HFr::zero(), power = HFr::one();
      std::vector<HFr> coeff;
      for (size_t b : active) {
        claim += claims[b] * power;
        coeff.push_back(power);
        power *= lam;
      }
      std::vector<HFr> x, evals;
      if (resident.layer(h, coeff, y, claim, tr, x, evals)) {
        c.route.v[RouteStats::RESIDENT_LAYERS]++;
        tr.write_field_elements(evals);
        HFr mu = tr.squeeze_challenge();
        x.push_back(mu);
        y = x;
        for (size_t k = 0; k < active.size(); k++) {
          const size_t b = active[k];
          const HFr &l = evals[2 * k], &r = evals[2 * k + 1];
          claims[b] = l + mu * (r - l);
          if (num_vars[b] == h + 1) {
            res.claims[b] = claims[b];
            res.points[b] = y;
// ... 104 lines not shown
```

### halo2-lasso_amd/csrc/host.hpp

```cpp
#pragma once
#include <string.h>
#include <functional>
#include <map>
#include <mutex>
#include <vector>
#include "dev.hpp"
#include "ff_host.hpp"

namespace lh {

const char* get_last_error();

typedef host::Fr HFr;
typedef host::G1Affine HG1;

static inline Fr dev(const HFr& f) {
  Fr r;
  memcpy(&r, &f, 32);
  return r;
}
static inline HFr hst(const Fr& f) {
  HFr r;
  memcpy(&r, &f, 32);
  return r;
// ... 95 lines not shown
  Fr odd, s2, s3;
};
struct ScU32Terms {
  struct Poly {
    std::vector<const uint32_t*> col;
    std::vector<size_t> len;
    std::vector<Fr> w;
  };
  std::vector<Poly> polys;
};
struct ScOptions {
  bool sum_is_exact = false;
  bool sharded = false;
  const ScRwPairs* rw = nullptr;
  const ScU32* u32 = nullptr;
  const ScU32Terms* u32_terms = nullptr;
};
SumCheckResult sum_check_prove(Ctx&, int prover_kind, size_t num_vars, const lh_sop& expr, const Fr* const* d_polys,
                               size_t num_polys, const HFr* ys, size_t num_ys, const HFr& sum, Transcript& tr,
                               const ScOptions& opt = ScOptions());

const Fr* eq_half_lookup(Ctx&, const HFr* y, size_t num_vars, bool sharded = false);
const Fr* eq_half_get(Ctx&, const HFr* y, size_t num_vars, bool sharded = false);
struct EqHalfScope {
  Ctx& c;
  size_t mark;
  explicit EqHalfScope(Ctx& c_) : c(c_), mark(c_.eq_half_cache.size()) {}
  ~EqHalfScope() { c.eq_half_cache.resize(mark); }
};

typedef std::function<void(const Fr* const*, Fr* const*, const Fr&, bool, size_t, Fr*)> RoundFn;
struct EqFactoring {
  struct One {
    size_t table;
    const HFr* y;
    std::vector<const Fr*> level;
    HFr S, S_prev;
    std::vector<HFr> q;
  };
  std::vector<One> eqs;
  bool per_term = false;
  bool trusted_claim = false;
  bool untrusted = false;
  std::vector<HFr> inv_1my;
  HFr c;
  HFr add_const;
  HFr kappa = HFr::one(), lin0 = HFr::zero(), lin1 = HFr::zero();
  std::function<bool(bool bind, size_t size)> streams;
  std::function<void(const Fr* const* in, Fr* const* out, const Fr& r, bool bind, size_t size, size_t round, int points,
                     Fr* out_host)>
      round;
  std::function<bool(const std::vector<const Fr*>& cur, bool bind, const HFr& r_prev, size_t n0, size_t round, const HFr& claim,
                     Transcript& tr, SumCheckResult& res)>
      resident_tail;
};
SumCheckResult sum_check_loop(Ctx&, int prover_kind, size_t num_vars, int degree, std::vector<const Fr*> cur,
                              const std::vector<char>& used, size_t num_polys, const HFr& sum, Transcript& tr,
                              bool sharded, const RoundFn& round_fn, const ScRound* tail_rd = nullptr,
                              EqFactoring* ef = nullptr);
SumCheckResult sum_check_prove_expr(Ctx&, size_t num_vars, const lh_expr& expr, const Fr* const* d_polys,
                                    size_t num_polys, const HFr* challenges, size_t num_challenges, const HFr* ys,
                                    size_t num_ys, const HFr& sum, Transcript& tr, bool sharded = false);

std::vector<HFr> evaluate_polys(Ctx&, const Fr* const* d_polys, size_t count, size_t num_vars, const HFr* point, bool sharded);
void comm_sum_fr(Ctx&, HFr* v, size_t n);
void comm_sum_points(Ctx&, HG1* pts, size_t n);
void comm_gather_tables(Ctx&, const Fr* local_block, size_t count, size_t n_local, size_t block, Fr* const* out);
void comm_gather_concat(Ctx&, const Fr* local, size_t n_local, Fr* out);
void eq_xy_shard(Ctx&, const Shard&, const HFr* y, size_t num_vars, size_t first, Fr* out_local);

struct FracSumCheckResult {
  std::vector<HFr> p_xs, q_xs, x;
};
FracSumCheckResult prove_fractional_sum_check(Ctx&, size_t num_batching, size_t num_vars,
                                              const HFr* const* claimed_p_0s, const HFr* const* claimed_q_0s,
                                              const Fr* const* d_ps, const Fr* const* d_qs, Transcript& tr);
struct GrandProductResult {
  std::vector<HFr> roots, claims;
  std::vector<std::vector<HFr>> points;
};
GrandProductResult prove_grand_product(Ctx&, size_t num_trees, const Fr* const* d_leaves, const size_t* num_vars,
                                       Transcript& tr, const Fr* const* d_level_up = nullptr,
                                       const uint8_t* plus_one = nullptr,
                                       const std::function<void()>& trees_built = nullptr);

struct Srs {
  G1Affine* d_eqs = nullptr;
  size_t num_vars = 0;
  const G1Affine* eq(size_t k) const { return d_eqs + (((size_t)1 << k) - 1); }
  mutable std::vector<G1Affine*> shard_levels;
  mutable int shard_rank = -1;
  mutable size_t shard_R = 0, shard_j = 0;
  mutable std::map<size_t, HG1> level_sums;
  mutable std::map<size_t, HG1> shard_level_sums;
  struct WinTable {
    G1Affine* d = nullptr;
    uint32_t c = 0, W = 0;
  };
  mutable std::map<size_t, WinTable> win_tables;
};
const Srs::WinTable* srs_window_table(Ctx&, const Srs&, size_t level);
const G1Affine* srs_shard_level(Ctx&, const Srs&, size_t level);
Srs* mkzg_setup(Ctx&, const HFr* ss, size_t num_vars);
std::vector<HG1> mkzg_batch_commit(Ctx&, const Srs&, const Fr* const* d_polys, size_t num_polys, size_t num_vars);
std::vector<HG1> mkzg_batch_commit_u32(Ctx&, const Srs&, const uint32_t* const* d_polys, size_t num_polys,
                                       size_t num_vars);
struct SmallOpen;
HFr mkzg_open(Ctx&, const Srs&, const Fr* d_poly, size_t num_vars, const HFr* point, Transcript& tr,
              const SmallOpen* small = nullptr);
struct SmallLinear {
  std::vector<size_t> poly;
  std::vector<HFr> coeff;
};
struct SmallPoly {
  const uint32_t* ptr = nullptr;
  size_t len = 0;
  uint32_t bits = 0;
  const SmallLinear* linear = nullptr;
};
void mkzg_batch_open(Ctx&, const Srs&, size_t num_vars, const Fr* const* d_polys, size_t num_polys,
                     const HFr* points, size_t num_points, const lh_evaluation* evals, size_t num_evals,
                     Transcript& tr, const SmallPoly* small = nullptr);

struct SmallOpen {
  std::vector<SmallPoly> cols;
  std::vector<HFr> coef;
  std::vector<const Fr*> merged;
  std::vector<Fr> merged_w;
  std::function<void()> ensure_merged;
};
void open_precommit_start(Ctx&, const Srs&, size_t num_vars, const SmallPoly* small, size_t num_polys,
                          const lh_evaluation* evals, size_t num_evals);
void additive_batch_open(Ctx&, size_t num_vars, const Fr* const* d_polys, size_t num_polys, const HFr* points,
                         size_t num_points, const lh_evaluation* evals, size_t num_evals, Transcript& tr,
                         const std::function<void(const Fr* g_prime, const HFr* point)>& open,
                         const SmallPoly* small = nullptr,
                         const std::function<void(const Fr* g_prime, const HFr* point, const SmallOpen&)>& open_small = nullptr);

struct USrs {
  G1Affine* d_powers = nullptr;
  size_t size = 0;
};
USrs* ukzg_setup(Ctx&, const HFr& s, size_t poly_size);
std::vector<HG1> zeromorph_batch_commit(Ctx&, const USrs&, size_t poly_size, const Fr* const* d_polys, size_t num_polys,
                                        size_t num_vars);
void zeromorph_open(Ctx&, const USrs&, size_t poly_size, const Fr* d_poly, size_t num_vars, const HFr* point,
                    Transcript& tr);
void zeromorph_batch_open(Ctx&, const USrs&, size_t poly_size, size_t num_vars, const Fr* const* d_polys,
                          size_t num_polys, const HFr* points, size_t num_points, const lh_evaluation* evals,
                          size_t num_evals, Transcript& tr, const SmallPoly* small = nullptr);
std::pair<HFr, std::vector<HFr>> zeromorph_scalars(const HFr& y, const HFr& x, const HFr& z, const HFr* u, size_t n);
struct ZmVerifierParams;
ZmVerifierParams* zeromorph_vp_setup(const HFr& s, size_t param_size, size_t poly_size);
ZmVerifierParams* zeromorph_vp_new(const lh_g1& g1, const lh_g2& g2, const lh_g2& s_g2, const lh_g2& s_offset_g2);
void zeromorph_vp_export(const ZmVerifierParams&, lh_g1* g1, lh_g2* g2, lh_g2* s_g2, lh_g2* s_offset_g2);
void zeromorph_vp_free(ZmVerifierParams*);
void zeromorph_verify(const ZmVerifierParams&, const HG1& comm, const HFr* point, size_t num_vars, const HFr& eval,
                      Transcript& tr);
void zeromorph_batch_verify(const ZmVerifierParams&, size_t num_vars, const HG1* comms, size_t num_comms,
                            const HFr* points, size_t num_points, const lh_evaluation* evals, size_t num_evals,
                            Transcript& tr);

struct UPoly {
  const Fr* d;
  size_t len;
};
std::vector<HG1> ukzg_batch_commit(Ctx&, const USrs&, size_t poly_size, const UPoly* polys, size_t num_polys);
// ... 181 lines not shown
```

### halo2-lasso_amd/csrc/kernels_poly.hip

```cpp
#include <hip/hip_runtime.h>
#include <string.h>
#include <algorithm>
#include "dev.hpp"
#include "ff_host.hpp"
#include "reduce.cuh"
#include "resident.cuh"
#include "wide.cuh"

namespace lh {

static inline dim3 grid_for(size_t n, int block = 256, size_t cap = 4096) {
  size_t g = (n + block - 1) / block;
  if (g < 1) g = 1;
  if (g > cap) g = cap;
  return dim3((unsigned)g);
}
#define GSTRIDE(i, n) \
  for (size_t i = (size_t)blockIdx.x * blockDim.x + threadIdx.x; i < (n); i += (size_t)gridDim.x * blockDim.x)

__global__ void fr_from_u64_kernel(const uint64_t* __restrict__ in, size_t n, Fr* __restrict__ out) {
  GSTRIDE(i, n) out[i] = from_u64<FrParams>(in[i]);
}
__global__ void fr_from_u32_kernel(const uint32_t* __restrict__ in, size_t n, Fr* __restrict__ out) {
  GSTRIDE(i, n) out[i] = from_u64<FrParams>(in[i]);
// ... 816 lines not shown
  __shared__ Fr lds[4];
  __shared__ int is_last;
  Fr acc = Fr::zero();
  GSTRIDE(i, entries) {
    const uint4 a = ((const uint4*)col)[i];
    Wide t = Wide::zero();
    wide_mac(t, k.w[0], a.x), wide_mac(t, k.w[1], a.y), wide_mac(t, k.w[2], a.z), wide_mac(t, k.w[3], a.w);
    const Fr v = wide_redc(t);
    out[i] = v;
    if (i & 1) acc = add(acc, mul(v, eq_level[i >> 1]));
  }
  acc = block_reduce_sum(acc, lds);
  if (gridDim.x == 1) {
    if (threadIdx.x == 0) {
      fin.out_host[0] = acc;
      publish_round(fin, 1);
    }
    return;
  }
  if (threadIdx.x == 0) fin_put(fin, partials, blockIdx.x, acc);
  if (!fin_ticket(fin, &is_last)) return;
  Fr a2 = Fr::zero();
  for (uint32_t i = threadIdx.x; i < gridDim.x; i += blockDim.x) a2 = add(a2, fin_get(fin, partials, i));
  a2 = block_reduce_sum(a2, lds);
  if (threadIdx.x == 0) {
    fin.out_host[0] = a2;
    publish_round(fin, 1);
  }
}
void k_sc_round_u32_bind2(Ctx& c, const uint32_t* col, const Fr* eq_level, const Fr& r0, const Fr& r1, size_t size, Fr* out,
                          Fr* out_host) {
  LH_REQUIRE(size >= 1 && !c.sc_redirect, LH_ERR_ARG, "sc_round_u32_bind2: bad shape");
  const uint32_t seq = c.next_seq();
  ArenaScope scope(c.arena);
  const size_t entries = 2 * size;
  const size_t g = std::min<size_t>((entries + 255) / 256, (size_t)c.num_cus * 8);
  Fr* partials = c.arena.alloc_n<Fr>(g);
  const ScFinishArgs fin = c.finish_for((uint32_t)g, out_host, seq, 32.0 * (double)entries);
  host::Fr h0, h1;
  const host::Fr one = host::Fr::one();
  memcpy(&h0, &r0, sizeof(h0));
  memcpy(&h1, &r1, sizeof(h1));
  const host::Fr w[4] = {(one - h1) * (one - h0), (one - h1) * h0, h1 * (one - h0), h1 * h0};
  U32Bind2 k;
  for (int i = 0; i < 4; i++) {
    Fr d;
    memcpy(&d, &w[i], sizeof(d));
    k.w[i] = prescale_r(d);
  }
  {
    ProfScope ps(c, "sc_round_u32<bind2>", 64.0 * (double)entries, 1.2 * (double)entries, (double)size);
    hipLaunchKernelGGL(sc_round_u32_bind2_kernel, dim3((unsigned)g), dim3(256), 0, c.stream, col, eq_level, k, entries, out, partials, fin);
  }
  c.wait_round(seq);
}

__global__ void tree_up_kernel(const Fr* __restrict__ in, size_t half, Fr* __restrict__ out) {
  GSTRIDE(i, half) out[i] = mul(in[i], in[half + i]);
}
__global__ void tree_up_multi_kernel(PtrPack p, size_t half) {
  const Fr* __restrict__ in = p.in[blockIdx.y];
  Fr* __restrict__ out = p.out[blockIdx.y];
  GSTRIDE(i, half) out[i] = mul(in[i], in[half + i]);
}
void k_tree_up_multi(Ctx& c, const Fr* const* in, Fr* const* out, size_t count, size_t half) {
  ProfScope ps(c, "tree_up", 96.0 * half * count, 1.0 * half * count, (double)half * count);
  if (!half) return;
  for (size_t base = 0; base < count; base += SC_MAX_TABLES) {
    size_t k = count - base < (size_t)SC_MAX_TABLES ? count - base : (size_t)SC_MAX_TABLES;
    PtrPack p;
    for (size_t i = 0; i < k; i++) {
      p.in[i] = in[base + i];
      p.out[i] = out[base + i];
    }
    dim3 g = grid_for(half);
    g.y = (unsigned)k;
    hipLaunchKernelGGL(tree_up_multi_kernel, g, 256, 0, c.stream, p, half);
  }
}
void k_tree_up(Ctx& c, const Fr* in, size_t half, Fr* out) {
  ProfScope ps(c, "tree_up", 96.0 * half, 1.0 * half, (double)half);
  if (half) hipLaunchKernelGGL(tree_up_kernel, grid_for(half), 256, 0, c.stream, in, half, out);
}
constexpr int TREE_SMALL = 9;
struct TreeTops {
  const Fr* in[SC_MAX_TABLES];
  Fr* out[SC_MAX_TABLES];
  int H[SC_MAX_TABLES];
};
__global__ __launch_bounds__(256) void tree_top_kernel(TreeTops t) {
  __shared__ Fr a[1 << TREE_SMALL];
  __shared__ Fr b[1 << (TREE_SMALL - 1)];
  const Fr* __restrict__ in = t.in[blockIdx.x];
  Fr* __restrict__ out = t.out[blockIdx.x];
  const int H = t.H[blockIdx.x];
  if (H <= 0) return;
  int half = 1 << H;
  for (int i = threadIdx.x; i < half; i += blockDim.x) {
    Fr v = mul(in[i], in[half + i]);
    a[i] = v;
    out[(half - 2) + i] = v;
  }
  __syncthreads();
  Fr* cur = a;
  Fr* nxt = b;
  for (int h = H - 2; h >= 0; h--) {
    half = 1 << (h + 1);
    for (int i = threadIdx.x; i < half; i += blockDim.x) {
      Fr v = mul(cur[i], cur[half + i]);
      nxt[i] = v;
      out[(half - 2) + i] = v;
    }
    __syncthreads();
    Fr* tmp = cur;
    cur = nxt;
    nxt = tmp;
  }
}
void k_tree_tops(Ctx& c, const Fr* const* in, Fr* const* out, const int* H, size_t count) {
  LH_REQUIRE(count <= (size_t)SC_MAX_TABLES, LH_ERR_ARG, "tree_tops: too many trees");
  if (!count) return;
  TreeTops t;
  for (size_t i = 0; i < count; i++) {
    LH_REQUIRE(H[i] <= TREE_SMALL, LH_ERR_ARG, "tree_tops: level too large");
    t.in[i] = in[i];
    t.out[i] = out[i];
    t.H[i] = H[i];
  }
  ProfScope ps(c, "tree_tops", 0, 0, (double)count);
  hipLaunchKernelGGL(tree_top_kernel, dim3((unsigned)count), dim3(256), 0, c.stream, t);
}

__global__ void frac_up_kernel(const Fr* __restrict__ p, const Fr* __restrict__ q, size_t half, Fr* __restrict__ vp,
                               Fr* __restrict__ vq) {
  GSTRIDE(i, half) {
    Fr pl = p[i], pr = p[half + i], ql = q[i], qr = q[half + i];
    vp[i] = add(mul(pl, qr), mul(pr, ql));
    vq[i] = mul(ql, qr);
  }
}
void k_frac_up(Ctx& c, const Fr* p, const Fr* q, size_t half, Fr* vp, Fr* vq) {
  ProfScope ps(c, "frac_up", 192.0 * half, 3.0 * half, (double)half);
  if (half) hipLaunchKernelGGL(frac_up_kernel, grid_for(half), 256, 0, c.stream, p, q, half, vp, vq);
}

__global__ void quotient_step_kernel(const Fr* __restrict__ rem, size_t half, Fr x, Fr* __restrict__ q,
                                     Fr* __restrict__ rem_out) {
  GSTRIDE(i, half) {
    Fr lo = rem[i], hi = rem[half + i];
    Fr d = sub(hi, lo);
    if (q) q[i] = d;
    rem_out[i] = add(lo, mul(d, x));
  }
}
void k_quotient_step(Ctx& c, const Fr* rem, size_t half, const Fr& x, Fr* q, Fr* rem_out) {
  ProfScope ps(c, "quotient_step", 128.0 * half, 1.0 * half, (double)half);
  if (half) hipLaunchKernelGGL(quotient_step_kernel, grid_for(half), 256, 0, c.stream, rem, half, x, q, rem_out);
}

__device__ __forceinline__ uint32_t subtable_entry(int kind, uint32_t m, uint32_t bits) {
  uint32_t h = bits >> 1;
  uint32_t x = m >> h, y = m & ((1u << h) - 1u);
  return kind == LH_SUBTABLE_IDENTITY ? m : kind == LH_SUBTABLE_AND ? (x & y) : (x ^ y);
}

constexpr uint32_t UNPERM_WINDOW_LOG = 15;
// ... 338 lines not shown
}
__global__ void lasso_output_small_kernel(LassoGSmall g, size_t n, uint32_t* __restrict__ a) {
  GSTRIDE(i, n) {
    uint32_t acc = 0;
    for (uint32_t t = 0; t < g.num_terms; t++) acc += g.coeff[t] * g.e[g.fac[t]][i];
    a[i] = acc;
  }
}
void k_lasso_output_small(Ctx& c, const LassoGSmall& g, size_t n, uint32_t* a) {
  ProfScope ps(c, "lasso_output", 4.0 * n * (g.num_terms + 1), 0.0, (double)n);
  if (n) hipLaunchKernelGGL(lasso_output_small_kernel, grid_for(n), 256, 0, c.stream, g, n, a);
}
void k_lasso_output(Ctx& c, const LassoG& g, size_t n, Fr* a) {
  ProfScope ps(c, "lasso_output", 36.0 * n, 2.0 * n, (double)n);
  if (n) hipLaunchKernelGGL(lasso_output_kernel, grid_for(n), 256, 0, c.stream, g, n, a);
}

__global__ void or_u32_kernel(const uint32_t* const* __restrict__ cols, size_t n, uint32_t* __restrict__ out) {
  const uint32_t* col = cols[blockIdx.y];
  uint32_t acc = 0;
  for (size_t i = (size_t)blockIdx.x * blockDim.x + threadIdx.x; i < n; i += (size_t)gridDim.x * blockDim.x) acc |= col[i];
  for (int off = 32; off > 0; off >>= 1) acc |= __shfl_xor(acc, off, 64);
  if ((threadIdx.x & 63) == 0 && acc) atomicOr(&out[blockIdx.y], acc);
}
void k_or_u32(Ctx& c, const uint32_t* const* cols, size_t count, size_t n, uint32_t* out_host) {
  if (!count) return;
  ArenaScope scope(c.arena);
  const uint32_t** d_cols = (const uint32_t**)c.arena.alloc(count * sizeof(uint32_t*));
  uint32_t* d_out = c.arena.alloc_n<uint32_t>(count);
  void* stage = c.pin(count * sizeof(uint32_t*));
  memcpy(stage, cols, count * sizeof(uint32_t*));
  LH_HIP(hipMemcpyAsync(d_cols, stage, count * sizeof(uint32_t*), hipMemcpyHostToDevice, c.stream));
  LH_HIP(hipMemsetAsync(d_out, 0, count * sizeof(uint32_t), c.stream));
  if (n)
    hipLaunchKernelGGL(or_u32_kernel, dim3((unsigned)std::min<size_t>((n + 255) / 256, 256), (unsigned)count), dim3(256), 0,
                       c.stream, d_cols, n, d_out);
  c.d2h(out_host, d_out, count * sizeof(uint32_t));
}
__global__ void fill_u32_kernel(uint32_t* __restrict__ out, uint32_t value, size_t n) {
  GSTRIDE(i, n) out[i] = value;
}
void k_fill_u32(Ctx& c, uint32_t* out, uint32_t value, size_t n) {
  if (n) hipLaunchKernelGGL(fill_u32_kernel, grid_for(n), 256, 0, c.stream, out, value, n);
}
__global__ void delta_u32_kernel(const uint32_t* __restrict__ col, size_t len, size_t half, uint64_t offset,
                                 uint32_t* __restrict__ out_lo, uint32_t* __restrict__ out_hi) {
  GSTRIDE(i, half) {
    const uint64_t lo = i < len ? col[i] : 0u, hi = i + half < len ? col[i + half] : 0u;
    const uint64_t v = hi + offset - lo;
    if (out_hi) {
      out_lo[i] = (uint32_t)(v & 0xffffu);
      out_hi[i] = (uint32_t)(v >> 16);
    } else {
      out_lo[i] = (uint32_t)v;
    }
  }
}
void k_delta_u32(Ctx& c, const uint32_t* col, size_t len, size_t half, uint64_t offset, uint32_t* out_lo, uint32_t* out_hi) {
  if (half)
    hipLaunchKernelGGL(delta_u32_kernel, grid_for(half), 256, 0, c.stream, col, len, half, offset, out_lo, out_hi);
}
__global__ void pack_u32_kernel(const uint32_t* __restrict__ a, const uint32_t* __restrict__ b, uint32_t shift, size_t n,
                                uint32_t* __restrict__ out) {
  GSTRIDE(i, n) out[i] = a[i] | (b[i] << shift);
}
void k_pack_u32(Ctx& c, const uint32_t* a, const uint32_t* b, uint32_t shift, size_t n, uint32_t* out) {
  if (n) hipLaunchKernelGGL(pack_u32_kernel, grid_for(n), 256, 0, c.stream, a, b, shift, n, out);
}

__global__ void lasso_rw_leaves_kernel(const uint32_t* __restrict__ dim, const uint32_t* __restrict__ e,
                                       const uint32_t* __restrict__ ts, size_t n, Fr gamma_r, Fr gamma2_r, Fr one_r, Fr tau,
                                       Fr* __restrict__ rs, Fr* __restrict__ ws) {
  const Fr one = Fr::one();
  GSTRIDE(i, n) {
    Wide t = Wide::zero();
    wide_mac(t, gamma2_r, dim[i]);
    wide_mac(t, gamma_r, e[i]);
    wide_mac(t, one_r, ts[i]);
    Fr h = sub(wide_redc(t), tau);
    rs[i] = h;
    ws[i] = add(h, one);
  }
}
__global__ void lasso_rw_leaves_up_kernel(const uint32_t* __restrict__ dim, const uint32_t* __restrict__ e,
                                          const uint32_t* __restrict__ ts, size_t half, Fr gamma_r, Fr gamma2_r, Fr one_r,
                                          Fr tau, Fr* __restrict__ rs, Fr* __restrict__ ws, Fr* __restrict__ rs_up,
                                          Fr* __restrict__ ws_up) {
  const Fr one = Fr::one();
  GSTRIDE(i, half) {
    Fr h[2];
#pragma unroll
    for (int k = 0; k < 2; k++) {
      const size_t j = i + (k ? half : 0);
      Wide t = Wide::zero();
      wide_mac(t, gamma2_r, dim[j]);
      wide_mac(t, gamma_r, e[j]);
      wide_mac(t, one_r, ts[j]);
      h[k] = sub(wide_redc(t), tau);
      rs[j] = h[k];
    }
    const Fr w0 = add(h[0], one), w1 = add(h[1], one);
    if (ws) {
      ws[i] = w0;
      ws[i + half] = w1;
    }
    rs_up[i] = mul(h[0], h[1]);
    ws_up[i] = mul(w0, w1);
  }
}
void k_lasso_rw_leaves_up(Ctx& c, const uint32_t* dim, const uint32_t* e, const uint32_t* ts, size_t n, const Fr& gamma,
                          const Fr& gamma2, const Fr& tau, Fr* rs, Fr* ws, Fr* rs_up, Fr* ws_up) {
  ProfScope ps(c, "lasso_rw_leaves", (12.0 + (ws ? 64.0 : 32.0) + 32.0) * n, 6.0 * n, (double)n);
  if (n >= 2)
    hipLaunchKernelGGL(lasso_rw_leaves_up_kernel, grid_for(n / 2), 256, 0, c.stream, dim, e, ts, n / 2, prescale_r(gamma),
                       prescale_r(gamma2), prescale_r(Fr::one()), tau, rs, ws, rs_up, ws_up);
}
void k_lasso_rw_leaves(Ctx& c, const uint32_t* dim, const uint32_t* e, const uint32_t* ts, size_t n, const Fr& gamma,
                       const Fr& gamma2, const Fr& tau, Fr* rs, Fr* ws) {
  ProfScope ps(c, "lasso_rw_leaves", (12.0 + 64.0) * n, 5.0 * n, (double)n);
  if (n)
    hipLaunchKernelGGL(lasso_rw_leaves_kernel, grid_for(n), 256, 0, c.stream, dim, e, ts, n, prescale_r(gamma),
                       prescale_r(gamma2), prescale_r(Fr::one()), tau, rs, ws);
}
__global__ void lasso_if_leaves_kernel(int kind, uint32_t bits, const uint32_t* __restrict__ final_cts, size_t m,
                                       Fr gamma, Fr gamma2, Fr tau, Fr* __restrict__ init, Fr* __restrict__ fin) {
  GSTRIDE(i, m) {
    Fr a = mul(from_u64<FrParams>(i), gamma2);
    Fr v = mul(from_u64<FrParams>(subtable_entry(kind, (uint32_t)i, bits)), gamma);
    Fr h = sub(add(a, v), tau);
    init[i] = h;
    fin[i] = add(h, from_u64<FrParams>(final_cts[i]));
  }
}
void k_lasso_if_leaves(Ctx& c, int subtable, uint32_t chunk_bits, const uint32_t* final_cts, size_t m,
                       const Fr& gamma, const Fr& gamma2, const Fr& tau, Fr* init, Fr* fin) {
  ProfScope ps(c, "lasso_if_leaves", (4.0 + 64.0) * m, 5.0 * m, (double)m);
  if (m)
    hipLaunchKernelGGL(lasso_if_leaves_kernel, grid_for(m), 256, 0, c.stream, subtable, chunk_bits, final_cts, m,
                       gamma, gamma2, tau, init, fin);
}

}
```

### halo2-lasso_amd/csrc/lasso.cpp

```cpp
#include <algorithm>
#include <chrono>
#include "host.hpp"

namespace lh {

static double now_ms() {
  using namespace std::chrono;
  return duration<double, std::milli>(steady_clock::now().time_since_epoch()).count();
}

void lasso_write_commitments(Transcript& tr, const std::vector<HG1>& comms) {
  LH_REQUIRE(comms.size() < 64, LH_ERR_ARG, "lasso: too many commitments for the identity mask");
  uint64_t mask = 0;
  for (size_t i = 0; i < comms.size(); i++)
    if (comms[i].is_identity()) mask |= (uint64_t)1 << i;
  tr.write_field_element(HFr::from_u64(mask));
  for (const HG1& cm : comms)
    if (!cm.is_identity()) tr.write_commitment(cm);
}

std::vector<HG1> lasso_read_commitments(Transcript& tr, size_t count) {
  LH_REQUIRE(count < 64, LH_ERR_ARG, "lasso: too many commitments for the identity mask");
  const HFr m = tr.read_field_element();
  uint64_t canon[4];
// ... 187 lines not shown
  Fr a_sums[4];
  bool have_a_sums = false;
  if (a_small && n >= 2) {
    const Fr* eq_half = eq_half_get(c, cl.r.data(), n, shn);
    if (!a && linear_g && !shn && n >= 3) {
      k_inner_products_small_quads(c, a_small, eq_half, N / 4, a_sums);
      const HFr r0 = cl.r[0];
      cl.v = (HFr::one() - r0) * hst(a_sums[0]) + r0 * hst(a_sums[1]);
      have_a_sums = true;
    } else {
      k_inner_products_small_half(c, &a_small, 1, eq_half, N / 2, dev(cl.r[0]), (Fr*)&cl.v);
    }
    sum_ranks(&cl.v, 1);
  } else if (a_small) {
    ArenaScope scope(c.arena);
    Fr* eq = c.arena.alloc_n<Fr>(N);
    k_eq_xy(c, (const Fr*)cl.r.data(), n, eq);
    k_inner_products_small(c, &a_small, 1, eq, N, (Fr*)&cl.v);
  } else {
    cl.v = evaluate_polys(c, &a, 1, n, cl.r.data(), shn)[0];
  }
  tr.write_field_element(cl.v);
  SumCheckResult sc;
  if (linear_g) {
    {
      ArenaScope scope(c.arena);
      const Fr* a_tab = a;
      ScU32 u32;
      ScOptions so;
      so.sum_is_exact = true, so.sharded = shn;
      if (!a_tab) {
        a_tab = c.arena.alloc_n<Fr>(N);
        u32.col = a_small;
        u32.have_sums = have_a_sums;
        if (have_a_sums) u32.odd = a_sums[1], u32.s2 = a_sums[2], u32.s3 = a_sums[3];
        so.u32 = &u32;
      }
      lh_sop one_term;
      memset(&one_term, 0, sizeof(one_term));
      one_term.global_eq = 0;
      one_term.num_terms = 1;
      const HFr one = HFr::one();
      memcpy(&one_term.coeff[0], &one, 32);
      one_term.num_factors[0] = 1;
      one_term.factor[0][0] = 0;
      sc = sum_check_prove(c, LH_SC_EVALUATIONS, n, one_term, &a_tab, 1, cl.r.data(), 1, cl.v, tr, so);
    }
    std::vector<const uint32_t*> cols(w.E.begin(), w.E.end());
    sc.evals.assign(alpha, HFr::zero());
    if (n >= 2) {
      const Fr* eq_half = eq_half_get(c, sc.challenges.data(), n, shn);
      k_inner_products_small_half(c, cols.data(), alpha, eq_half, N / 2, dev(sc.challenges[0]), (Fr*)sc.evals.data());
      sum_ranks(sc.evals.data(), alpha);
    } else {
      ArenaScope scope(c.arena);
      Fr* eq = c.arena.alloc_n<Fr>(N);
      k_eq_xy(c, (const Fr*)sc.challenges.data(), n, eq);
      k_inner_products_small(c, cols.data(), alpha, eq, N, (Fr*)sc.evals.data());
    }
  } else {
    lh_sop surge;
    memset(&surge, 0, sizeof(surge));
    surge.global_eq = 0;
    surge.num_terms = tb.num_terms;
    for (uint32_t m = 0; m < tb.num_terms; m++) {
      surge.coeff[m] = tb.g_coeff[m];
      surge.num_factors[m] = tb.g_num_factors[m];
      for (int k = 0; k < LH_SC_MAX_FACTORS; k++) surge.factor[m][k] = tb.g_factor[m][k];
    }
    ScOptions so;
    so.sum_is_exact = true, so.sharded = shn;
    sc = sum_check_prove(c, LH_SC_EVALUATIONS, n, surge, E_fr, alpha, cl.r.data(), 1, cl.v, tr, so);
  }
  cl.r_z = sc.challenges;
  cl.e_rz = sc.evals;
  tr.write_field_elements(sc.evals);
  if (lap) lap(2);

  HFr gamma = tr.squeeze_challenge();
  HFr tau = tr.squeeze_challenge();
  HFr gamma2 = gamma * gamma;
  {
    ArenaScope scope(c.arena);
    std::vector<const Fr*> leaves(4 * alpha), level_up(4 * alpha, nullptr);
    std::vector<size_t> depths(4 * alpha);
    std::vector<uint8_t> plus_one(4 * alpha, 0);
    const bool fused_up = n >= 12 && (!shn || sh.sharded(n - 1)), ws_implicit = fused_up && n > l;
    for (size_t i = 0; i < alpha; i++) {
      size_t j = tb.memory_chunk[i];
      Fr* rs = c.arena.alloc_n<Fr>(N);
      Fr* ws = ws_implicit ? nullptr : c.arena.alloc_n<Fr>(N);
      Fr* in = c.arena.alloc_n<Fr>(M);
      Fr* fi = c.arena.alloc_n<Fr>(M);
      if (fused_up) {
        Fr* rs_up = c.arena.alloc_n<Fr>(N / 2);
        Fr* ws_up = c.arena.alloc_n<Fr>(N / 2);
        k_lasso_rw_leaves_up(c, d_dims[j], w.E[i], w.rts[j], N, dev(gamma), dev(gamma2), dev(tau), rs, ws, rs_up, ws_up);
        level_up[2 * i] = rs_up, level_up[2 * i + 1] = ws_up;
      } else {
        k_lasso_rw_leaves(c, d_dims[j], w.E[i], w.rts[j], N, dev(gamma), dev(gamma2), dev(tau), rs, ws);
      }
      k_lasso_if_leaves(c, (int)tb.memory_subtable[i], (uint32_t)l, w.fcs[j], M, dev(gamma), dev(gamma2), dev(tau), in, fi);
      leaves[2 * i] = rs, leaves[2 * i + 1] = ws;
      plus_one[2 * i + 1] = 1;
      leaves[2 * alpha + 2 * i] = in, leaves[2 * alpha + 2 * i + 1] = fi;
      depths[2 * i] = depths[2 * i + 1] = n;
      depths[2 * alpha + 2 * i] = depths[2 * alpha + 2 * i + 1] = l;
    }
    if (lap) lap(3);
    GrandProductResult gp = prove_grand_product(c, 4 * alpha, leaves.data(), depths.data(), tr, level_up.data(), plus_one.data(), trees_built);
    cl.r_N = gp.points[0];
    cl.r_M = gp.points[2 * alpha];
  }
  if (lap) lap(4);

  const Fr* eq_half_n = n >= 2 ? eq_half_get(c, cl.r_N.data(), n, shn) : nullptr;
  {
    ArenaScope scope(c.arena);
    std::vector<const uint32_t*> at_n;
    for (size_t j = 0; j < cc; j++) at_n.push_back(d_dims[j]);
    for (size_t j = 0; j < cc; j++) at_n.push_back(w.rts[j]);
    for (size_t i = 0; i < alpha; i++) at_n.push_back(w.E[i]);
    cl.ev_n.resize(at_n.size());
    Fr* eq = c.arena.alloc_n<Fr>(eq_half_n ? M : std::max(N, M));
    if (eq_half_n) {
      k_inner_products_small_half(c, at_n.data(), at_n.size(), eq_half_n, N / 2, dev(cl.r_N[0]), (Fr*)cl.ev_n.data());
      sum_ranks(cl.ev_n.data(), cl.ev_n.size());
    } else {
      k_eq_xy(c, (const Fr*)cl.r_N.data(), n, eq);
      k_inner_products_small(c, at_n.data(), at_n.size(), eq, N, (Fr*)cl.ev_n.data());
    }
    std::vector<const uint32_t*> at_l(w.fcs.begin(), w.fcs.end());
    cl.ev_l.resize(cc);
    k_eq_xy(c, (const Fr*)cl.r_M.data(), l, eq);
    k_inner_products_small(c, at_l.data(), cc, eq, M, (Fr*)cl.ev_l.data());
  }
  tr.write_field_elements(cl.ev_n);
  tr.write_field_elements(cl.ev_l);
  if (lap) lap(5);
  return cl;
}

void lasso_prove(Ctx& c, const Pcs& pcs, const lh_lasso_table& tb, size_t n, const uint32_t* const* d_dims,
                 Transcript& tr) {
  lasso_check_table(tb);
  const size_t cc = tb.num_chunks, l = tb.chunk_bits, alpha = tb.num_memories;
  LH_REQUIRE(n >= 1 && n < 31, LH_ERR_ARG, "lasso: need at least one variable");
  if (n > pcs.max_vars || l > pcs.max_vars)
    throw Error(LH_ERR_INVALID_PCS_PARAM, "Too many variates of poly to commit");
  const Shard sh(c);
  const bool shn = sh.on;
  if (shn) {
    LH_REQUIRE(pcs.shard_bases != nullptr, LH_ERR_ARG, "sharded prove: implemented for multilinear KZG");
    LH_REQUIRE(sh.j >= 1 && l <= sh.j + sh.rho, LH_ERR_ARG,
               "sharded prove: need shard_bit + rho >= chunk_bits (subtables replicated)");
    LH_REQUIRE(sh.sharded(n) && n >= l, LH_ERR_ARG, "sharded prove: 2^num_vars lookups are too few to shard");
  }
  const size_t nv = std::max(n, l), NV = (size_t)1 << (nv - sh.rho);
  const size_t N = (size_t)1 << (n - sh.rho), M = (size_t)1 << l;
  const double t0 = now_ms();
  double* ph = c.lasso_ms;
  for (int k = 0; k < 8; k++)
    if (!c.phase_ev[k]) LH_HIP(hipEventCreate(&c.phase_ev[k]));
  c.phase_ev_pending = false;
  LH_HIP(hipEventRecord(c.phase_ev[0], c.stream));
  c.comm_phase = 0;
  struct PhaseGuard {
    Ctx& c;
    ~PhaseGuard() { c.comm_phase = 7; }
  } phase_guard{c};
  auto lap = [&](int idx) {
    LH_HIP(hipEventRecord(c.phase_ev[idx + 1], c.stream));
    c.comm_phase = idx + 1;
  };

  ArenaScope scope(c.arena);
  EqHalfScope eq_scope(c);
  c.route = RouteStats();
  std::vector<uint32_t> count_ors(cc, 0);
  Fr* a = nullptr;
  uint32_t* a_small = nullptr;
  LassoColumns w = lasso_witness_columns(c, tb, n, d_dims, &a, &a_small, n >= (size_t)knob(Knob::MSM_SLAB_LOG));
  std::vector<uint32_t*>&rts = w.rts, &fcs = w.fcs, &E = w.E;
  lap(0);
  tr.common_field_element(HFr::from_u64(n));
  tr.common_field_element(HFr::from_u64(l));
  tr.common_field_element(HFr::from_u64(cc));
  tr.common_field_element(HFr::from_u64(alpha));
  {
    const G1Affine* bases = shn ? pcs.shard_bases(nv) : pcs.commit_bases(nv);
    bool linear_g = true;
    for (uint32_t m = 0; m < tb.num_terms; m++) linear_g = linear_g && tb.g_num_factors[m] == 1;
    const size_t total = 1 + 3 * cc + alpha;
// ... 216 lines not shown
```

### include/lasso_hip.h

```cpp
#ifndef LASSO_HIP_H
#define LASSO_HIP_H

#include <stddef.h>
#include <stdint.h>

#ifdef __cplusplus
extern "C" {
#endif

typedef struct { uint64_t l[4]; } lh_fr;
typedef struct { uint64_t x[4], y[4]; } lh_g1;

typedef int lh_status;
#define LH_OK 0
#define LH_ERR_INVALID_SUMCHECK (-1)
#define LH_ERR_INVALID_PCS_PARAM (-2)
#define LH_ERR_INVALID_PCS_OPEN (-3)
#define LH_ERR_INVALID_SNARK (-4)
#define LH_ERR_SERIALIZATION (-5)
#define LH_ERR_TRANSCRIPT (-6)
#define LH_ERR_DEVICE (-7)
#define LH_ERR_ARG (-8)

typedef struct lh_ctx lh_ctx;
// ... 6 lines not shown
lh_status lh_ctx_sync(lh_ctx* ctx);
void* lh_ctx_stream(lh_ctx* ctx);
lh_status lh_alloc(lh_ctx* ctx, size_t bytes, void** d_out);
lh_status lh_free(lh_ctx* ctx, void* d_ptr);
lh_status lh_upload(lh_ctx* ctx, void* d_dst, const void* src, size_t bytes);
lh_status lh_download(lh_ctx* ctx, void* dst, const void* d_src, size_t bytes);

typedef struct lh_transcript {
  void* user;
  int (*write_field_element)(void* user, const lh_fr* fe);
  int (*common_field_element)(void* user, const lh_fr* fe);
  int (*squeeze_challenge)(void* user, lh_fr* out);
  int (*write_commitment)(void* user, const lh_g1* pt);
  int (*common_commitment)(void* user, const lh_g1* pt);
  int (*read_field_element)(void* user, lh_fr* out);
  int (*read_commitment)(void* user, lh_g1* out);
} lh_transcript;

lh_status lh_keccak_transcript_new(lh_transcript** out);
void lh_keccak_transcript_free(lh_transcript* t);
lh_status lh_keccak_transcript_proof(lh_transcript* t, const uint8_t** bytes, size_t* len);
lh_status lh_keccak_transcript_from_proof(const uint8_t* proof, size_t len, lh_transcript** out);
lh_status lh_keccak_transcript_remaining(lh_transcript* t, size_t* out);

lh_status lh_fr_from_u64(lh_ctx*, const uint64_t* d_in, size_t n, lh_fr* d_out);
lh_status lh_fr_from_u32(lh_ctx*, const uint32_t* d_in, size_t n, lh_fr* d_out);
lh_status lh_fr_to_repr(lh_ctx*, const lh_fr* d_in, size_t n, uint8_t* d_out32);
lh_status lh_fr_from_repr(lh_ctx*, const uint8_t* d_in32, size_t n, lh_fr* d_out);
lh_status lh_fr_add(lh_ctx*, const lh_fr* d_a, const lh_fr* d_b, size_t n, lh_fr* d_out);
lh_status lh_fr_sub(lh_ctx*, const lh_fr* d_a, const lh_fr* d_b, size_t n, lh_fr* d_out);
lh_status lh_fr_mul(lh_ctx*, const lh_fr* d_a, const lh_fr* d_b, size_t n, lh_fr* d_out);
lh_status lh_fr_mul_chain(lh_ctx*, const lh_fr* d_a, const lh_fr* d_b, size_t n, int iters, lh_fr* d_out);
lh_status lh_fr_batch_invert(lh_ctx*, const lh_fr* d_in, size_t n, lh_fr* d_out);

lh_status lh_fix_var(lh_ctx*, const lh_fr* d_in, size_t n_in, const lh_fr* x, lh_fr* d_out);
lh_status lh_eq_xy(lh_ctx*, const lh_fr* y, size_t num_vars, lh_fr* d_out);
lh_status lh_evaluate(lh_ctx*, const lh_fr* const* d_polys, size_t num_polys, size_t num_vars,
                      const lh_fr* point, lh_fr* out_evals);
lh_status lh_lincomb(lh_ctx*, const lh_fr* const* d_polys, const lh_fr* w, size_t num_polys,
                     size_t n, lh_fr* d_out);

#define LH_SC_MAX_TERMS 48
#define LH_SC_MAX_FACTORS 4
typedef struct lh_sop {
  uint32_t num_terms;
  int32_t global_eq;
  lh_fr coeff[LH_SC_MAX_TERMS];
  uint8_t num_factors[LH_SC_MAX_TERMS];
  uint8_t factor[LH_SC_MAX_TERMS][LH_SC_MAX_FACTORS];
} lh_sop;

#define LH_SC_EVALUATIONS 0
#define LH_SC_COEFFICIENTS 1
lh_status lh_sumcheck_prove(lh_ctx*, int prover_kind, size_t num_vars, const lh_sop* expr,
                            const lh_fr* const* d_polys, size_t num_polys,
                            const lh_fr* ys, size_t num_ys,
                            const lh_fr* sum, lh_transcript* t,
                            lh_fr* out_challenges, lh_fr* out_evals);

#define LH_EX_CONSTANT 0
#define LH_EX_IDENTITY 1
#define LH_EX_LAGRANGE 2
#define LH_EX_EQ_XY 3
#define LH_EX_POLYNOMIAL 4
#define LH_EX_CHALLENGE 5
#define LH_EX_NEGATED 6
#define LH_EX_SUM 7
#define LH_EX_PRODUCT 8
#define LH_EX_SCALED 9
typedef struct lh_expr_node { uint32_t op; int32_t a, b; uint32_t reserved; lh_fr scalar; } lh_expr_node;
typedef struct lh_expr { const lh_expr_node* nodes; size_t num_nodes; } lh_expr;
lh_status lh_sumcheck_prove_expr(lh_ctx*, size_t num_vars, const lh_expr* expr, const lh_fr* const* d_polys,
                                 size_t num_polys, const lh_fr* challenges, size_t num_challenges,
                                 const lh_fr* ys, size_t num_ys, const lh_fr* sum, lh_transcript* t,
                                 lh_fr* out_challenges, lh_fr* out_evals);

lh_status lh_gkr_fractional_prove(lh_ctx*, size_t num_batching, size_t num_vars,
                                  const lh_fr* const* claimed_p_0s, const lh_fr* const* claimed_q_0s,
                                  const lh_fr* const* d_ps, const lh_fr* const* d_qs,
                                  lh_transcript* t, lh_fr* out_p_xs, lh_fr* out_q_xs, lh_fr* out_x);
lh_status lh_grand_product_prove(lh_ctx*, size_t num_trees, const lh_fr* const* d_leaves,
                                 const size_t* num_vars, lh_transcript* t, lh_fr* out_roots,
                                 lh_fr* out_claims, lh_fr* out_points);

lh_status lh_msm(lh_ctx*, const lh_fr* d_scalars, const lh_g1* d_bases, size_t n, lh_g1* out);
lh_status lh_msm_u32(lh_ctx*, const uint32_t* d_scalars, const lh_g1* d_bases, size_t n, lh_g1* out);

typedef struct lh_srs lh_srs;
lh_status lh_mkzg_setup(lh_ctx*, const lh_fr* ss, size_t num_vars, lh_srs** out);
lh_status lh_srs_upload(lh_ctx*, const lh_g1* eqs_flat, size_t num_vars, lh_srs** out);
lh_status lh_srs_download(lh_ctx*, const lh_srs*, lh_g1* eqs_flat);
size_t lh_srs_num_vars(const lh_srs*);
void lh_srs_free(lh_ctx*, lh_srs*);
lh_status lh_mkzg_commit(lh_ctx*, const lh_srs*, const lh_fr* d_poly, size_t num_vars, lh_g1* out);
lh_status lh_mkzg_batch_commit(lh_ctx*, const lh_srs*, const lh_fr* const* d_polys, size_t num_polys,
                               size_t num_vars, lh_g1* out_comms);
lh_status lh_mkzg_open(lh_ctx*, const lh_srs*, const lh_fr* d_poly, size_t num_vars,
                       const lh_fr* point, lh_transcript* t, lh_fr* out_eval);
typedef struct lh_evaluation { uint32_t poly, point; lh_fr value; } lh_evaluation;
lh_status lh_mkzg_batch_open(lh_ctx*, const lh_srs*, size_t num_vars,
                             const lh_fr* const* d_polys, size_t num_polys,
                             const lh_fr* points, size_t num_points,
                             const lh_evaluation* evals, size_t num_evals, lh_transcript* t);

#define LH_SUBTABLE_IDENTITY 0
#define LH_SUBTABLE_AND 1
#define LH_SUBTABLE_XOR 2
#define LH_LASSO_MAX_CHUNKS 8
#define LH_LASSO_MAX_MEMORIES 16
#define LH_LASSO_MAX_TERMS 16
typedef struct lh_lasso_table {
  uint32_t num_chunks;
  uint32_t chunk_bits;
  uint32_t num_memories;
  uint32_t memory_chunk[LH_LASSO_MAX_MEMORIES];
  uint32_t memory_subtable[LH_LASSO_MAX_MEMORIES];
  uint32_t num_terms;
  lh_fr g_coeff[LH_LASSO_MAX_TERMS];
  uint8_t g_num_factors[LH_LASSO_MAX_TERMS];
  uint8_t g_factor[LH_LASSO_MAX_TERMS][LH_SC_MAX_FACTORS];
} lh_lasso_table;
lh_status lh_lasso_prove(lh_ctx*, const lh_srs*, const lh_lasso_table*, size_t num_vars,
                         const uint32_t* const* d_dims, lh_transcript* t);

#define LH_LASSO_NUM_PHASES 9
lh_status lh_lasso_last_timing(lh_ctx*, double* out_ms);

lh_status lh_ctx_set_option(lh_ctx*, const char* name, int64_t value);
lh_status lh_ctx_get_option(lh_ctx*, const char* name, int64_t* out);
#define LH_LASSO_ROUTE_WORDS 24
typedef struct lh_lasso_route {
  uint32_t open_small_depth;
  uint32_t open_small_passes;
  uint32_t eq_factored_rounds;
  uint32_t standard_rounds;
  uint32_t rw_leaf_rounds;
  uint32_t resident_tails;
  uint32_t resident_rounds;
  uint32_t packed_ts_pairs;
  uint32_t derived_commitments;
  uint32_t sorted_dim_reuse;
  uint32_t sharded_rounds;
  uint32_t shard_exchanges;
  uint32_t window_table_jobs;
  uint32_t open_precommit;
  uint32_t resident_layers;
  uint32_t pp_folds;
  uint32_t msm_half_batches;
  uint32_t reserved[7];
} lh_lasso_route;
lh_status lh_lasso_last_route(lh_ctx*, lh_lasso_route* out);

typedef struct lh_comm {
  int rank, size;
  void* user;
  int (*all_gather)(void* user, const void* send, void* recv, size_t bytes_per_rank);
  int (*all_gather_device)(void* user, const void* d_send, void* d_recv, size_t bytes_per_rank, void* hip_stream);
} lh_comm;
lh_status lh_ctx_set_comm(lh_ctx*, const lh_comm* comm, size_t shard_bit);
#define LH_RCCL_UNIQUE_ID_BYTES 128
lh_status lh_rccl_unique_id(uint8_t out[LH_RCCL_UNIQUE_ID_BYTES]);
lh_status lh_ctx_set_comm_rccl(lh_ctx*, int rank, int size, const uint8_t unique_id[LH_RCCL_UNIQUE_ID_BYTES],
                               size_t shard_bit);
lh_status lh_ctx_set_comm_loopback(lh_ctx*, int rank, int size, size_t shard_bit);
lh_status lh_ctx_comm_stats(lh_ctx*, uint64_t out[2]);
lh_status lh_ctx_comm_phase_stats(lh_ctx*, uint64_t out[16], int reset);
lh_status lh_ctx_memory_stats(lh_ctx*, uint64_t out[4]);
lh_status lh_ctx_host_cpus(lh_ctx*, char* bus_id, size_t bus_id_cap, char* cpulist, size_t cpulist_cap);
lh_status lh_lasso_prove_sharded(lh_ctx*, const lh_srs*, const lh_lasso_table*, size_t num_vars,
                                 const uint32_t* const* d_dims_local, lh_transcript* t);

typedef struct lh_hp_lookup {
  const lh_expr* inputs;
  const lh_expr* tables;
  size_t width;
} lh_hp_lookup;
#define LH_HP_LASSO_MAX_COMMITMENTS 63
typedef struct lh_hp_lasso_lookup {
  lh_lasso_table table;
  size_t output_poly;
  size_t chunk_polys[LH_LASSO_MAX_CHUNKS];
} lh_hp_lasso_lookup;
typedef struct lh_hp_param {
  size_t num_vars;
  size_t num_instance_polys;
  const size_t* num_instances;
  size_t num_preprocess_polys;
  const void* const* d_preprocess_polys;
  size_t num_witness_polys;
  size_t num_challenges;
  size_t num_lookups;
  const lh_hp_lookup* lookups;
  size_t num_permutation_polys;
  const size_t* permutation_poly_index;
  const void* const* d_permutation_polys;
  size_t num_permutation_z_polys;
  lh_expr expression;
  size_t num_lasso_lookups;
  const lh_hp_lasso_lookup* lasso_lookups;
} lh_hp_param;
lh_status lh_hyperplonk_prove(lh_ctx*, const lh_srs*, const lh_hp_param*, const lh_fr* const* instances,
                              const lh_fr* const* d_witness_polys, lh_transcript* t);

lh_status lh_shard_extract(lh_ctx*, const void* d_global, size_t n_local, size_t shard_bit, size_t rho, size_t rank,
                           size_t elem_bytes, void* d_local);
lh_status lh_hyperplonk_prove_sharded(lh_ctx*, const lh_srs*, const lh_hp_param*, const lh_fr* const* instances,
                                      const lh_fr* const* d_witness_polys_local, lh_transcript* t);

typedef struct lh_hp_circuit {
  void* user;
  int (*synthesize)(void* user, size_t round, const lh_fr* challenges, size_t num_challenges,
                    const void** d_out_polys, size_t num_out);
} lh_hp_circuit;
lh_status lh_hyperplonk_prove_phases(lh_ctx*, const lh_srs*, const lh_hp_param*, size_t num_phases,
                                     const size_t* num_witness_polys, const size_t* num_challenges,
                                     const lh_fr* const* instances, const lh_hp_circuit* circuit, lh_transcript* t);

typedef struct lh_g2 { uint64_t x_c0[4], x_c1[4], y_c0[4], y_c1[4]; } lh_g2;
typedef struct lh_mkzg_vp lh_mkzg_vp;
lh_status lh_mkzg_vp_setup(const lh_fr* ss, size_t num_vars, lh_mkzg_vp** out);
lh_status lh_mkzg_vp_new(const lh_g1* g1, const lh_g2* g2, const lh_g2* ss, size_t num_vars, lh_mkzg_vp** out);
lh_status lh_mkzg_vp_export(const lh_mkzg_vp*, lh_g1* g1, lh_g2* g2, lh_g2* ss);
size_t lh_mkzg_vp_num_vars(const lh_mkzg_vp*);
void lh_mkzg_vp_free(lh_mkzg_vp*);
lh_status lh_pairing_check(const lh_g1* ps, const lh_g2* qs, size_t n, int* out_is_identity);
lh_status lh_mkzg_verify(const lh_mkzg_vp*, const lh_g1* comm, const lh_fr* point, size_t num_vars,
                         const lh_fr* eval, lh_transcript* t);
lh_status lh_mkzg_batch_verify(const lh_mkzg_vp*, size_t num_vars, const lh_g1* comms, size_t num_comms,
                               const lh_fr* points, size_t num_points, const lh_evaluation* evals,
                               size_t num_evals, lh_transcript* t);
lh_status lh_sumcheck_verify(int prover_kind, size_t num_vars, size_t degree, const lh_fr* sum,
                             lh_transcript* t, lh_fr* out_eval, lh_fr* out_x);
// ... 208 lines not shown
```

Measured before the change: 56.86 ms.

## Fuse two product-tree levels per pass in leaves and grand-product trees

The read/write leaf kernel can now also produce the second tree level (quarter-size products), and the grand-product tree builder computes two levels per kernel pass when not sharded and no trees join at the next level. This removes one full read of each intermediate level from memory and halves the number of tree-up launches. The ws_up computation is also rewritten as r + h0 + h1 + 1 to replace one field multiplication with additions. In exchange there is more arena memory live at once and more branching in the level builder, and the sharded path keeps the old one-level behaviour.

```diff
diff --git a/bindings/rust/src/sys.rs b/bindings/rust/src/sys.rs
--- a/bindings/rust/src/sys.rs
+++ b/bindings/rust/src/sys.rs
@@ -177,7 +177,9 @@
     pub resident_layers: u32,
     pub pp_folds: u32,
     pub msm_half_batches: u32,
-    pub reserved: [u32; 7],
+    pub leaves_two_levels: u32,
+    pub tree_two_level_passes: u32,
+    pub reserved: [u32; 5],
 }
 
 extern "C" {
diff --git a/halo2-lasso_amd/__init__.py b/halo2-lasso_amd/__init__.py
--- a/halo2-lasso_amd/__init__.py
+++ b/halo2-lasso_amd/__init__.py
@@ -441,6 +441,31 @@
         pts.append(flat[off:off + p.num_vars])
         off += p.num_vars
     return _fr_list(roots, B), list(zip(_fr_list(claims, B), pts))
+
+
+def product_tree_levels(ctx, leaves):
+    B = len(leaves)
+    nv = (C.c_size_t * max(B, 1))(*[p.num_vars for p in leaves])
+    outs = [ctx.alloc(32 * max((1 << p.num_vars) - 2, 1)) for p in leaves]
+    _check(ctx.lib.lh_product_tree_levels(ctx.h, B, _ptr_array(leaves), nv, _ptr_array(outs)))
+    res = []
+    for p, o in zip(leaves, outs):
+        flat = frs_from_bytes(o.read(32 * ((1 << p.num_vars) - 2))) if p.num_vars > 1 else []
+        res.append([flat[(2 << h) - 2:(4 << h) - 2] for h in range(p.num_vars - 1)])
+    return res
+
+
+def lasso_rw_leaves_up(ctx, dim, e, ts, gamma, tau, two_levels, with_ws=True):
+    import array
+    n = len(dim)
+    cols = [ctx.upload(array.array("I", c).tobytes()) for c in (dim, e, ts)]
+    names = ["rs", "ws", "rs_up", "ws_up", "rs_up2", "ws_up2"]
+    sizes = [n, n, n // 2, n // 2, n // 4, n // 4]
+    want = [True, with_ws, True, True, two_levels, two_levels]
+    bufs = [ctx.alloc(32 * k) if w else None for k, w in zip(sizes, want)]
+    _check(ctx.lib.lh_lasso_rw_leaves_up(ctx.h, cols[0].ptr, cols[1].ptr, cols[2].ptr, n, _fr_array([gamma]), _fr_array([tau]),
+                                         *[b.ptr if b else None for b in bufs]))
+    return {k: frs_from_bytes(b.read(32 * m)) if b else None for k, b, m in zip(names, bufs, sizes)}
 
 
 def variable_base_msm(ctx, scalars, bases, n=None):
@@ -1466,7 +1491,8 @@
 
 ROUTE_FIELDS = ["open_small_depth", "open_small_passes", "eq_factored_rounds", "standard_rounds", "rw_leaf_rounds",
                 "resident_tails", "resident_rounds", "packed_ts_pairs", "derived_commitments", "sorted_dim_reuse",
-                "sharded_rounds", "shard_exchanges", "window_table_jobs", "open_precommit", "resident_layers", "pp_folds", "msm_half_batches"]
+                "sharded_rounds", "shard_exchanges", "window_table_jobs", "open_precommit", "resident_layers", "pp_folds", "msm_half_batches",
+                "leaves_two_levels", "tree_two_level_passes"]
 
 
 def lasso_last_route(ctx):
diff --git a/halo2-lasso_amd/_ffi.py b/halo2-lasso_amd/_ffi.py
--- a/halo2-lasso_amd/_ffi.py
+++ b/halo2-lasso_amd/_ffi.py
@@ -168,6 +168,8 @@
                                           C.POINTER(lh_fr), C.POINTER(lh_fr), C.POINTER(lh_fr)]),
     "lh_grand_product_prove": (C.c_int, [_P, _SZ, C.POINTER(_P), C.POINTER(_SZ), C.POINTER(lh_transcript),
                                          C.POINTER(lh_fr), C.POINTER(lh_fr), C.POINTER(lh_fr)]),
+    "lh_product_tree_levels": (C.c_int, [_P, _SZ, C.POINTER(_P), C.POINTER(_SZ), C.POINTER(_P)]),
+    "lh_lasso_rw_leaves_up": (C.c_int, [_P, _P, _P, _P, _SZ, C.POINTER(lh_fr), C.POINTER(lh_fr), _P, _P, _P, _P, _P, _P]),
     "lh_msm": (C.c_int, [_P, _P, _P, _SZ, C.POINTER(lh_g1)]),
     "lh_msm_u32": (C.c_int, [_P, _P, _P, _SZ, C.POINTER(lh_g1)]),
     "lh_mkzg_setup": (C.c_int, [_P, C.POINTER(lh_fr), _SZ, C.POINTER(_P)]),
diff --git a/halo2-lasso_amd/csrc/capi.cpp b/halo2-lasso_amd/csrc/capi.cpp
--- a/halo2-lasso_amd/csrc/capi.cpp
+++ b/halo2-lasso_amd/csrc/capi.cpp
@@ -425,6 +425,44 @@
   LH_CATCH
 }
 
+lh_status lh_product_tree_levels(lh_ctx* ctx, size_t num_trees, const lh_fr* const* d_leaves, const size_t* num_vars,
+                                 lh_fr* const* d_out) {
+  LH_TRY NEED_CTX(ctx);
+  NEED(num_vars);
+  NEED_N(d_leaves, num_trees);
+  NEED_N(d_out, num_trees);
+  for (size_t b = 0; b < num_trees; b++) {
+    NEED(d_leaves[b]);
+    LH_REQUIRE(d_out[b] != nullptr || num_vars[b] == 1, LH_ERR_ARG, "null argument: d_out[b]");
+  }
+  product_tree_levels(ctx->c, num_trees, (const Fr* const*)d_leaves, num_vars, (Fr* const*)d_out);
+  LH_CATCH
+}
+lh_status lh_lasso_rw_leaves_up(lh_ctx* ctx, const uint32_t* d_dim, const uint32_t* d_e, const uint32_t* d_ts, size_t n,
+                                const lh_fr* gamma, const lh_fr* tau, lh_fr* d_rs, lh_fr* d_ws, lh_fr* d_rs_up,
+                                lh_fr* d_ws_up, lh_fr* d_rs_up2, lh_fr* d_ws_up2) {
+  LH_TRY NEED_CTX(ctx);
+  NEED(d_dim);
+  NEED(d_e);
+  NEED(d_ts);
+  NEED(gamma);
+  NEED(tau);
+  NEED(d_rs);
+  NEED(d_rs_up);
+  NEED(d_ws_up);
+  LH_REQUIRE(is_pow2(n) && n >= 2, LH_ERR_ARG, "lasso_rw_leaves_up: columns must have 2^k >= 2 entries");
+  LH_REQUIRE((d_rs_up2 != nullptr) == (d_ws_up2 != nullptr) && (!d_rs_up2 || n >= 4), LH_ERR_ARG,
+             "lasso_rw_leaves_up: the second level needs both trees and >= 4 entries");
+  HFr g, t;
+  memcpy(&g, gamma, 32);
+  memcpy(&t, tau, 32);
+  const HFr g2 = g * g;
+  k_lasso_rw_leaves_up(ctx->c, d_dim, d_e, d_ts, n, dev(g), dev(g2), dev(t), (Fr*)d_rs, (Fr*)d_ws, (Fr*)d_rs_up,
+                       (Fr*)d_ws_up, (Fr*)d_rs_up2, (Fr*)d_ws_up2);
+  ctx->c.sync();
+  LH_CATCH
+}
+
 lh_status lh_msm(lh_ctx* ctx, const lh_fr* d_scalars, const lh_g1* d_bases, size_t n, lh_g1* out) {
   LH_TRY NEED_CTX(ctx);
   NEED(out);
diff --git a/halo2-lasso_amd/csrc/dev.hpp b/halo2-lasso_amd/csrc/dev.hpp
--- a/halo2-lasso_amd/csrc/dev.hpp
+++ b/halo2-lasso_amd/csrc/dev.hpp
@@ -128,7 +128,8 @@
 struct RouteStats {
   uint32_t v[LH_LASSO_ROUTE_WORDS] = {0};
   enum { OPEN_DEPTH, OPEN_PASSES, EF_ROUNDS, STD_ROUNDS, RW_ROUNDS, TAILS, TAIL_ROUNDS, PACKED_TS, DERIVED, SORTED_REUSE,
-         SHARDED_ROUNDS, SHARD_EXCHANGES, WIN_TABLE_JOBS, OPEN_PRECOMMIT, RESIDENT_LAYERS, PP_FOLDS, MSM_HALF_BATCHES };
+         SHARDED_ROUNDS, SHARD_EXCHANGES, WIN_TABLE_JOBS, OPEN_PRECOMMIT, RESIDENT_LAYERS, PP_FOLDS, MSM_HALF_BATCHES,
+         LEAVES_UP2, TREE_UP2 };
 };
 
 class HostWorker {
@@ -346,13 +347,15 @@
                      const size_t* sm_len, const Fr* wsm, size_t num_sm, size_t n, Fr* out);
 void k_tree_up(Ctx&, const Fr* in, size_t half, Fr* out);
 void k_tree_up_multi(Ctx&, const Fr* const* in, Fr* const* out, size_t count, size_t half);
+void k_tree_up2_multi(Ctx&, const Fr* const* in, Fr* const* out1, Fr* const* out2, size_t count, size_t q);
 void k_tree_tops(Ctx&, const Fr* const* in, Fr* const* out, const int* H, size_t count);
 void k_frac_up(Ctx&, const Fr* p, const Fr* q, size_t half, Fr* vp, Fr* vq);
 void k_quotient_step(Ctx&, const Fr* rem, size_t half, const Fr& x, Fr* q, Fr* rem_out);
 void k_lasso_rw_leaves(Ctx&, const uint32_t* dim, const uint32_t* e, const uint32_t* ts, size_t n,
                        const Fr& gamma, const Fr& gamma2, const Fr& tau, Fr* rs, Fr* ws);
 void k_lasso_rw_leaves_up(Ctx&, const uint32_t* dim, const uint32_t* e, const uint32_t* ts, size_t n, const Fr& gamma,
-                          const Fr& gamma2, const Fr& tau, Fr* rs, Fr* ws, Fr* rs_up, Fr* ws_up);
+                          const Fr& gamma2, const Fr& tau, Fr* rs, Fr* ws, Fr* rs_up, Fr* ws_up, Fr* rs_up2 = nullptr,
+                          Fr* ws_up2 = nullptr);
 void k_lasso_if_leaves(Ctx&, int subtable, uint32_t chunk_bits, const uint32_t* final_cts, size_t m,
                        const Fr& gamma, const Fr& gamma2, const Fr& tau, Fr* init, Fr* fin);
 void k_or_u32(Ctx&, const uint32_t* const* cols, size_t count, size_t n, uint32_t* out_host);
diff --git a/halo2-lasso_amd/csrc/gkr.cpp b/halo2-lasso_amd/csrc/gkr.cpp
--- a/halo2-lasso_amd/csrc/gkr.cpp
+++ b/halo2-lasso_amd/csrc/gkr.cpp
@@ -112,9 +112,78 @@
   return FracSumCheckResult{claimed_p, claimed_q, y};
 }
 
+static void build_product_levels(Ctx& c, size_t B, std::vector<std::vector<const Fr*>>& level, std::vector<size_t>& cur_h,
+                                 size_t small) {
+  const Shard sh(c);
+  size_t max_h = 0;
+  for (size_t b = 0; b < B; b++) max_h = std::max(max_h, cur_h[b]);
+  for (size_t h = max_h; h >= 1 && (h > small || sh.sharded(h + 1)); h--) {
+    std::vector<const Fr*> ins;
+    std::vector<Fr*> outs;
+    std::vector<size_t> who;
+    const bool in_sh = sh.sharded(h + 1), out_sh = sh.sharded(h);
+    const size_t half = (size_t)1 << (in_sh ? h - sh.rho : h);
+    bool joiners = false;
+    for (size_t b = 0; b < B; b++) {
+      joiners = joiners || cur_h[b] + 1 == h;
+      if (cur_h[b] != h) continue;
+      ins.push_back(level[b][h]);
+      who.push_back(b);
+    }
+    if (ins.empty()) continue;
+    const bool two = !sh.on && h >= small + 2 && !joiners;
+    for (size_t b : who) cur_h[b] = two ? h - 2 : h - 1;
+    if (two) {
+      std::vector<Fr*> outs2;
+      for (size_t k = 0; k < ins.size(); k++) {
+        outs.push_back(c.arena.alloc_n<Fr>(half));
+        outs2.push_back(c.arena.alloc_n<Fr>(half / 2));
+        level[who[k]][h - 1] = outs[k];
+        level[who[k]][h - 2] = outs2[k];
+      }
+      k_tree_up2_multi(c, ins.data(), outs.data(), outs2.data(), ins.size(), half / 2);
+      c.route.v[RouteStats::TREE_UP2]++;
+    } else if (in_sh && !out_sh) {
+      Fr* block = c.arena.alloc_n<Fr>(ins.size() * half);
+      std::vector<Fr*> rep(ins.size());
+      for (size_t k = 0; k < ins.size(); k++) {
+        outs.push_back(block + k * half);
+        rep[k] = c.arena.alloc_n<Fr>((size_t)1 << h);
+      }
+      k_tree_up_multi(c, ins.data(), outs.data(), ins.size(), half);
+      comm_gather_tables(c, block, ins.size(), half, half, rep.data());
+      c.route.v[RouteStats::SHARD_EXCHANGES]++;
+      for (size_t k = 0; k < ins.size(); k++) level[who[k]][h - 1] = rep[k];
+    } else {
+      for (size_t k = 0; k < ins.size(); k++) {
+        outs.push_back(c.arena.alloc_n<Fr>(half));
+        level[who[k]][h - 1] = outs.back();
+      }
+      k_tree_up_multi(c, ins.data(), outs.data(), ins.size(), half);
+    }
+  }
+}
+void product_tree_levels(Ctx& c, size_t B, const Fr* const* d_leaves, const size_t* num_vars, Fr* const* d_out) {
+  ArenaScope scope(c.arena);
+  std::vector<std::vector<const Fr*>> level(B);
+  std::vector<size_t> cur_h(B);
+  for (size_t b = 0; b < B; b++) {
+    LH_REQUIRE(num_vars[b] >= 1 && num_vars[b] < 32, LH_ERR_ARG, "product tree: every tree needs >= 2 leaves");
+    level[b].resize(num_vars[b]);
+    level[b][num_vars[b] - 1] = d_leaves[b];
+    cur_h[b] = num_vars[b] - 1;
+  }
+  build_product_levels(c, B, level, cur_h, 0);
+  for (size_t b = 0; b < B; b++)
+    for (size_t h = 0; h + 1 < num_vars[b]; h++)
+      LH_HIP(hipMemcpyAsync(d_out[b] + (((size_t)2 << h) - 2), level[b][h], ((size_t)2 << h) * sizeof(Fr),
+                            hipMemcpyDeviceToDevice, c.stream));
+  c.sync();
+}
+
 GrandProductResult prove_grand_product(Ctx& c, size_t B, const Fr* const* d_leaves, const size_t* num_vars,
                                        Transcript& tr, const Fr* const* d_level_up, const uint8_t* plus_one,
-                                       const std::function<void()>& trees_built) {
+                                       const std::function<void()>& trees_built, const Fr* const* d_level_up2) {
   LH_REQUIRE(B != 0, LH_ERR_ARG, "grand product: no trees");
   size_t max_depth = 0;
   for (size_t b = 0; b < B; b++) {
@@ -132,7 +201,6 @@
     std::vector<Fr*> top_out(B);
     std::vector<int> top_H(B);
     std::vector<size_t> cur_h(B);
-    size_t max_h = 0;
     for (size_t b = 0; b < B; b++) {
       level[b].resize(num_vars[b]);
       level[b][num_vars[b] - 1] = d_leaves[b];
@@ -140,42 +208,14 @@
       if (d_level_up && d_level_up[b] && h > SMALL && (!sh.on || sh.sharded(h))) {
         level[b][h - 1] = d_level_up[b];
         h--;
+        if (d_level_up2 && d_level_up2[b] && h > SMALL && !sh.on) {
+          level[b][h - 1] = d_level_up2[b];
+          h--;
+        }
       }
       cur_h[b] = h;
-      max_h = std::max(max_h, h);
-    }
-    for (size_t h = max_h; h >= 1 && (h > SMALL || sh.sharded(h + 1)); h--) {
-      std::vector<const Fr*> ins;
-      std::vector<Fr*> outs;
-      std::vector<size_t> who;
-      const bool in_sh = sh.sharded(h + 1), out_sh = sh.sharded(h);
-      const size_t half = (size_t)1 << (in_sh ? h - sh.rho : h);
-      for (size_t b = 0; b < B; b++) {
-        if (cur_h[b] != h) continue;
-        ins.push_back(level[b][h]);
-        who.push_back(b);
-        cur_h[b] = h - 1;
-      }
-      if (ins.empty()) continue;
-      if (in_sh && !out_sh) {
-        Fr* block = c.arena.alloc_n<Fr>(ins.size() * half);
-        std::vector<Fr*> rep(ins.size());
-        for (size_t k = 0; k < ins.size(); k++) {
-          outs.push_back(block + k * half);
-          rep[k] = c.arena.alloc_n<Fr>((size_t)1 << h);
-        }
-        k_tree_up_multi(c, ins.data(), outs.data(), ins.size(), half);
-        comm_gather_tables(c, block, ins.size(), half, half, rep.data());
-        c.route.v[RouteStats::SHARD_EXCHANGES]++;
-        for (size_t k = 0; k < ins.size(); k++) level[who[k]][h - 1] = rep[k];
-      } else {
-        for (size_t k = 0; k < ins.size(); k++) {
-          outs.push_back(c.arena.alloc_n<Fr>(half));
-          level[who[k]][h - 1] = outs.back();
-        }
-        k_tree_up_multi(c, ins.data(), outs.data(), ins.size(), half);
-      }
-    }
+    }
+    build_product_levels(c, B, level, cur_h, SMALL);
     for (size_t b = 0; b < B; b++) {
       const size_t h = cur_h[b];
       LH_REQUIRE(h <= SMALL && !sh.sharded(h + 1), LH_ERR_ARG, "grand product: internal level mismatch");
diff --git a/halo2-lasso_amd/csrc/host.hpp b/halo2-lasso_amd/csrc/host.hpp
--- a/halo2-lasso_amd/csrc/host.hpp
+++ b/halo2-lasso_amd/csrc/host.hpp
@@ -201,7 +201,9 @@
 GrandProductResult prove_grand_product(Ctx&, size_t num_trees, const Fr* const* d_leaves, const size_t* num_vars,
                                        Transcript& tr, const Fr* const* d_level_up = nullptr,
                                        const uint8_t* plus_one = nullptr,
-                                       const std::function<void()>& trees_built = nullptr);
+                                       const std::function<void()>& trees_built = nullptr,
+                                       const Fr* const* d_level_up2 = nullptr);
+void product_tree_levels(Ctx&, size_t num_trees, const Fr* const* d_leaves, const size_t* num_vars, Fr* const* d_out);
 
 struct Srs {
   G1Affine* d_eqs = nullptr;
diff --git a/halo2-lasso_amd/csrc/kernels_poly.hip b/halo2-lasso_amd/csrc/kernels_poly.hip
--- a/halo2-lasso_amd/csrc/kernels_poly.hip
+++ b/halo2-lasso_amd/csrc/kernels_poly.hip
@@ -922,6 +922,38 @@
   ProfScope ps(c, "tree_up", 96.0 * half, 1.0 * half, (double)half);
   if (half) hipLaunchKernelGGL(tree_up_kernel, grid_for(half), 256, 0, c.stream, in, half, out);
 }
+struct PtrPack2 {
+  const Fr* in[SC_MAX_TABLES];
+  Fr* out1[SC_MAX_TABLES];
+  Fr* out2[SC_MAX_TABLES];
+};
+__global__ void tree_up2_multi_kernel(PtrPack2 p, size_t q) {
+  const Fr* __restrict__ in = p.in[blockIdx.y];
+  Fr* __restrict__ out1 = p.out1[blockIdx.y];
+  Fr* __restrict__ out2 = p.out2[blockIdx.y];
+  GSTRIDE(i, q) {
+    const Fr lo = mul(in[i], in[2 * q + i]), hi = mul(in[q + i], in[3 * q + i]);
+    out1[i] = lo;
+    out1[q + i] = hi;
+    out2[i] = mul(lo, hi);
+  }
+}
+void k_tree_up2_multi(Ctx& c, const Fr* const* in, Fr* const* out1, Fr* const* out2, size_t count, size_t q) {
+  ProfScope ps(c, "tree_up", 224.0 * q * count, 3.0 * q * count, 3.0 * q * count);
+  if (!q) return;
+  for (size_t base = 0; base < count; base += SC_MAX_TABLES) {
+    size_t k = count - base < (size_t)SC_MAX_TABLES ? count - base : (size_t)SC_MAX_TABLES;
+    PtrPack2 p;
+    for (size_t i = 0; i < k; i++) {
+      p.in[i] = in[base + i];
+      p.out1[i] = out1[base + i];
+      p.out2[i] = out2[base + i];
+    }
+    dim3 g = grid_for(q);
+    g.y = (unsigned)k;
+    hipLaunchKernelGGL(tree_up2_multi_kernel, g, 256, 0, c.stream, p, q);
+  }
+}
 constexpr int TREE_SMALL = 9;
 struct TreeTops {
   const Fr* in[SC_MAX_TABLES];
@@ -1426,6 +1458,15 @@
     ws[i] = add(h, one);
   }
 }
+__device__ __forceinline__ Fr rw_fingerprint(const uint32_t* __restrict__ dim, const uint32_t* __restrict__ e,
+                                             const uint32_t* __restrict__ ts, size_t j, const Fr& gamma_r,
+                                             const Fr& gamma2_r, const Fr& one_r, const Fr& tau) {
+  Wide t = Wide::zero();
+  wide_mac(t, gamma2_r, dim[j]);
+  wide_mac(t, gamma_r, e[j]);
+  wide_mac(t, one_r, ts[j]);
+  return sub(wide_redc(t), tau);
+}
 __global__ void lasso_rw_leaves_up_kernel(const uint32_t* __restrict__ dim, const uint32_t* __restrict__ e,
                                           const uint32_t* __restrict__ ts, size_t half, Fr gamma_r, Fr gamma2_r, Fr one_r,
                                           Fr tau, Fr* __restrict__ rs, Fr* __restrict__ ws, Fr* __restrict__ rs_up,
@@ -1436,26 +1477,53 @@
 #pragma unroll
     for (int k = 0; k < 2; k++) {
       const size_t j = i + (k ? half : 0);
-      Wide t = Wide::zero();
-      wide_mac(t, gamma2_r, dim[j]);
-      wide_mac(t, gamma_r, e[j]);
-      wide_mac(t, one_r, ts[j]);
-      h[k] = sub(wide_redc(t), tau);
+      h[k] = rw_fingerprint(dim, e, ts, j, gamma_r, gamma2_r, one_r, tau);
       rs[j] = h[k];
-    }
-    const Fr w0 = add(h[0], one), w1 = add(h[1], one);
-    if (ws) {
-      ws[i] = w0;
-      ws[i + half] = w1;
-    }
-    rs_up[i] = mul(h[0], h[1]);
-    ws_up[i] = mul(w0, w1);
+      if (ws) ws[j] = add(h[k], one);
+    }
+    const Fr s = add(add(h[0], h[1]), one);
+    const Fr r = mul(h[0], h[1]);
+    rs_up[i] = r;
+    ws_up[i] = add(r, s);
+  }
+}
+__global__ void lasso_rw_leaves_up2_kernel(const uint32_t* __restrict__ dim, const uint32_t* __restrict__ e,
+                                           const uint32_t* __restrict__ ts, size_t q, Fr gamma_r, Fr gamma2_r, Fr one_r,
+                                           Fr tau, Fr* __restrict__ rs, Fr* __restrict__ ws, Fr* __restrict__ rs_up,
+                                           Fr* __restrict__ ws_up, Fr* __restrict__ rs_up2, Fr* __restrict__ ws_up2) {
+  const Fr one = Fr::one();
+  GSTRIDE(i, q) {
+    Fr r[2], w[2];
+#pragma unroll
+    for (int k = 0; k < 2; k++) {
+      Fr h[2];
+#pragma unroll
+      for (int m = 0; m < 2; m++) {
+        const size_t j = i + (size_t)(k + 2 * m) * q;
+        h[m] = rw_fingerprint(dim, e, ts, j, gamma_r, gamma2_r, one_r, tau);
+        rs[j] = h[m];
+        if (ws) ws[j] = add(h[m], one);
+      }
+      const Fr s = add(add(h[0], h[1]), one);
+      r[k] = mul(h[0], h[1]);
+      w[k] = add(r[k], s);
+      rs_up[i + k * q] = r[k];
+      ws_up[i + k * q] = w[k];
+    }
+    rs_up2[i] = mul(r[0], r[1]);
+    ws_up2[i] = mul(w[0], w[1]);
   }
 }
 void k_lasso_rw_leaves_up(Ctx& c, const uint32_t* dim, const uint32_t* e, const uint32_t* ts, size_t n, const Fr& gamma,
-                          const Fr& gamma2, const Fr& tau, Fr* rs, Fr* ws, Fr* rs_up, Fr* ws_up) {
-  ProfScope ps(c, "lasso_rw_leaves", (12.0 + (ws ? 64.0 : 32.0) + 32.0) * n, 6.0 * n, (double)n);
-  if (n >= 2)
+                          const Fr& gamma2, const Fr& tau, Fr* rs, Fr* ws, Fr* rs_up, Fr* ws_up, Fr* rs_up2, Fr* ws_up2) {
+  const bool two = rs_up2 != nullptr;
+  LH_REQUIRE(two == (ws_up2 != nullptr) && (!two || n >= 4), LH_ERR_ARG, "lasso_rw_leaves_up: bad second level");
+  ProfScope ps(c, "lasso_rw_leaves", (12.0 + (ws ? 64.0 : 32.0) + 32.0 + (two ? 16.0 : 0.0)) * n, (two ? 6.0 : 5.5) * n,
+               (double)n);
+  if (two)
+    hipLaunchKernelGGL(lasso_rw_leaves_up2_kernel, grid_for(n / 4), 256, 0, c.stream, dim, e, ts, n / 4, prescale_r(gamma),
+                       prescale_r(gamma2), prescale_r(Fr::one()), tau, rs, ws, rs_up, ws_up, rs_up2, ws_up2);
+  else if (n >= 2)
     hipLaunchKernelGGL(lasso_rw_leaves_up_kernel, grid_for(n / 2), 256, 0, c.stream, dim, e, ts, n / 2, prescale_r(gamma),
                        prescale_r(gamma2), prescale_r(Fr::one()), tau, rs, ws, rs_up, ws_up);
 }
diff --git a/halo2-lasso_amd/csrc/lasso.cpp b/halo2-lasso_amd/csrc/lasso.cpp
--- a/halo2-lasso_amd/csrc/lasso.cpp
+++ b/halo2-lasso_amd/csrc/lasso.cpp
@@ -293,10 +293,11 @@
   HFr gamma2 = gamma * gamma;
   {
     ArenaScope scope(c.arena);
-    std::vector<const Fr*> leaves(4 * alpha), level_up(4 * alpha, nullptr);
+    std::vector<const Fr*> leaves(4 * alpha), level_up(4 * alpha, nullptr), level_up2(4 * alpha, nullptr);
     std::vector<size_t> depths(4 * alpha);
     std::vector<uint8_t> plus_one(4 * alpha, 0);
     const bool fused_up = n >= 12 && (!shn || sh.sharded(n - 1)), ws_implicit = fused_up && n > l;
+    const bool fused_up2 = fused_up && !shn;
     for (size_t i = 0; i < alpha; i++) {
       size_t j = tb.memory_chunk[i];
       Fr* rs = c.arena.alloc_n<Fr>(N);
@@ -306,8 +307,13 @@
       if (fused_up) {
         Fr* rs_up = c.arena.alloc_n<Fr>(N / 2);
         Fr* ws_up = c.arena.alloc_n<Fr>(N / 2);
-        k_lasso_rw_leaves_up(c, d_dims[j], w.E[i], w.rts[j], N, dev(gamma), dev(gamma2), dev(tau), rs, ws, rs_up, ws_up);
+        Fr* rs_up2 = fused_up2 ? c.arena.alloc_n<Fr>(N / 4) : nullptr;
+        Fr* ws_up2 = fused_up2 ? c.arena.alloc_n<Fr>(N / 4) : nullptr;
+        k_lasso_rw_leaves_up(c, d_dims[j], w.E[i], w.rts[j], N, dev(gamma), dev(gamma2), dev(tau), rs, ws, rs_up, ws_up,
+                             rs_up2, ws_up2);
         level_up[2 * i] = rs_up, level_up[2 * i + 1] = ws_up;
+        level_up2[2 * i] = rs_up2, level_up2[2 * i + 1] = ws_up2;
+        if (fused_up2) c.route.v[RouteStats::LEAVES_UP2]++;
       } else {
         k_lasso_rw_leaves(c, d_dims[j], w.E[i], w.rts[j], N, dev(gamma), dev(gamma2), dev(tau), rs, ws);
       }
@@ -319,7 +325,8 @@
       depths[2 * alpha + 2 * i] = depths[2 * alpha + 2 * i + 1] = l;
     }
     if (lap) lap(3);
-    GrandProductResult gp = prove_grand_product(c, 4 * alpha, leaves.data(), depths.data(), tr, level_up.data(), plus_one.data(), trees_built);
+    GrandProductResult gp = prove_grand_product(c, 4 * alpha, leaves.data(), depths.data(), tr, level_up.data(), plus_one.data(), trees_built,
+                                                    level_up2.data());
     cl.r_N = gp.points[0];
     cl.r_M = gp.points[2 * alpha];
   }
diff --git a/include/lasso_hip.h b/include/lasso_hip.h
--- a/include/lasso_hip.h
+++ b/include/lasso_hip.h
@@ -112,6 +112,11 @@
 lh_status lh_grand_product_prove(lh_ctx*, size_t num_trees, const lh_fr* const* d_leaves,
                                  const size_t* num_vars, lh_transcript* t, lh_fr* out_roots,
                                  lh_fr* out_claims, lh_fr* out_points);
+lh_status lh_product_tree_levels(lh_ctx*, size_t num_trees, const lh_fr* const* d_leaves, const size_t* num_vars,
+                                 lh_fr* const* d_out);
+lh_status lh_lasso_rw_leaves_up(lh_ctx*, const uint32_t* d_dim, const uint32_t* d_e, const uint32_t* d_ts, size_t n,
+                                const lh_fr* gamma, const lh_fr* tau, lh_fr* d_rs, lh_fr* d_ws, lh_fr* d_rs_up,
+                                lh_fr* d_ws_up, lh_fr* d_rs_up2, lh_fr* d_ws_up2);
 
 lh_status lh_msm(lh_ctx*, const lh_fr* d_scalars, const lh_g1* d_bases, size_t n, lh_g1* out);
 lh_status lh_msm_u32(lh_ctx*, const uint32_t* d_scalars, const lh_g1* d_bases, size_t n, lh_g1* out);
@@ -177,7 +182,9 @@
   uint32_t resident_layers;
   uint32_t pp_folds;
   uint32_t msm_half_batches;
-  uint32_t reserved[7];
+  uint32_t leaves_two_levels;
+  uint32_t tree_two_level_passes;
+  uint32_t reserved[5];
 } lh_lasso_route;
 lh_status lh_lasso_last_route(lh_ctx*, lh_lasso_route* out);
 
```

Measured after the change: 56.75 ms, median of 2. No clear change (-0.2%).
